# Domingo1337/Chiaroscuro-RayTracer

Measured on AMD Instinct MI355X. Metric: Mray/s (primary+secondary) on sponza_crytek 1080p; 1/2/4/8-GPU scaling, higher is better.
Workload: dtype f32; 1 GPU; sponza_standin (Sponza-Crytek stand-in, ~261k tris) 1920x1080; k=6, tile=32, parallelism=tile-split x1, rays=7648053528, rays_answered_untraced=1312885262, layers_per_pass=32, trace_build=59, texture_bytes=0

## Files before the change

### chiaroscuro-raytracer_amd/chiaroscuro_amd/__init__.py

```python
from __future__ import annotations

import ctypes as C
import os
from pathlib import Path

import numpy as np

PKG_ROOT = Path(__file__).resolve().parent.parent
LIB_DIR = Path(os.environ["CHIARO_LIB_DIR"]) if os.environ.get("CHIARO_LIB_DIR") else PKG_ROOT / "lib"

CR_OK = 0
CR_ERRORS = {-1: "CR_E_INVALID", -2: "CR_E_HIP", -3: "CR_E_NOSCENE", -4: "CR_E_DEPTH", -5: "CR_E_OOM",
             -6: "CR_E_COMM"}
COMM_ID_BYTES = 128

f3 = C.c_float * 3


class CrCamera(C.Structure):
    _fields_ = [("eye", f3), ("left_upper", f3), ("dx", f3), ("dy", f3)]

    def as_array(self) -> np.ndarray:
        return np.array(list(self.eye) + list(self.left_upper) + list(self.dx) + list(self.dy), dtype=np.float32)

# ... 68 lines not shown
    a = np.ascontiguousarray(x, np.float32)
    out = np.zeros(a.shape, np.uint16)
    libs()[1].chiaro_float_to_half(_ptr(a), out.ctypes.data_as(C.POINTER(C.c_uint16)), a.size)
    return out


class CrKdNode(C.Structure):
    _fields_ = [("split", C.c_float), ("axis", C.c_uint32), ("child_or_first", C.c_uint32), ("count", C.c_uint32)]


class CrTexture(C.Structure):
    _fields_ = [("width", C.c_int32), ("height", C.c_int32), ("components", C.c_int32),
                ("data", C.POINTER(C.c_uint8))]


class CrSceneDesc(C.Structure):
    _fields_ = [("n_nodes", C.c_uint32), ("nodes", C.POINTER(CrKdNode)), ("n_refs", C.c_uint32),
                ("refs", C.POINTER(C.c_uint32)), ("max_depth", C.c_uint32), ("box_min", f3), ("box_max", f3),
                ("n_tris", C.c_uint32), ("tri_pos", C.POINTER(C.c_float)), ("tri_normal", C.POINTER(C.c_float)),
                ("tri_kd", C.POINTER(C.c_float)), ("tri_ke", C.POINTER(C.c_float)),
                ("tri_uv", C.POINTER(C.c_float)), ("tri_tex", C.POINTER(C.c_int32)),
                ("tri_emissive", C.POINTER(C.c_uint8)), ("n_lights", C.c_uint32),
                ("light_id", C.POINTER(C.c_uint32)), ("light_surface", C.POINTER(C.c_float)),
                ("n_textures", C.c_uint32), ("textures", C.POINTER(CrTexture))]


class ChiaroSceneInfo(C.Structure):
    _fields_ = [("xres", C.c_uint32), ("yres", C.c_uint32), ("samples", C.c_uint32),
                ("preview_height", C.c_uint32), ("leaf_size", C.c_uint32), ("seed", C.c_uint32),
                ("k", C.c_int32), ("using_preview", C.c_int32), ("VP", f3), ("LA", f3), ("UP", f3),
                ("background", f3), ("yview", C.c_float), ("exposure", C.c_float), ("n_invalid", C.c_uint32),
                ("obj_path", C.c_char * 1024), ("render_path", C.c_char * 1024), ("gpus", C.c_uint32)]


TRACE_KINDS = ("camera", "closest", "shadow", "tail")
DIAG_NAMES = ("rounds", "lanes", "distinct", "records", "maxcount", "lanetests", "fit64", "fit128",
              "urounds", "tests", "geomiss", "rep1", "rep4", "rep8")
PERF_NAMES = ("queries", "steps", "leaves", "masks", "tests", "vbytes", "sbytes", "waves",
              "drounds", "diters", "dlanes", "dtests")


class CrTraceStats(C.Structure):
    _fields_ = [("launches", C.c_uint64 * 4), ("ms", C.c_double * 4), ("inner", C.c_uint64 * 4),
                ("leaf", C.c_uint64 * 4), ("tritest", C.c_uint64 * 4), ("chunked_shades", C.c_uint64)]


class CrTonemapParams(C.Structure):
    _fields_ = [(n, C.c_float) for n in ("m", "s", "kl", "f", "defog", "gamma")]


class CrNoiseParams(C.Structure):
    _fields_ = [("threshold", C.c_float), ("floor", C.c_float)]


class CrNoiseStats(C.Structure):
    _fields_ = [("pixels", C.c_uint64), ("above", C.c_uint64), ("max_err", C.c_float), ("layers", C.c_uint32)]

    def as_dict(self) -> dict:
        return {"pixels": int(self.pixels), "above": int(self.above), "max_err": float(self.max_err),
                "layers": int(self.layers)}


def tonemap_params(exposure, defog=0.0, knee_low=0.0, knee_high=5.0, gamma=2.2) -> CrTonemapParams:
    t = CrTonemapParams()
    libs()[0].cr_tonemap_setup(exposure, defog, knee_low, knee_high, gamma, C.byref(t))
    return t


_hip = None
_host = None

HIP_SYMBOLS = ("cr_create", "cr_destroy", "cr_last_error", "cr_upload_scene", "cr_render", "cr_render_device",
               "cr_render_tiles_device", "cr_blend_tiles_device", "cr_tiles_for_rank", "cr_tile_origin", "cr_intersect",
               "cr_intersect_shadow", "cr_intersect_device", "cr_intersect_shadow_device", "cr_get_counters", "cr_last_kernel_ms", "cr_get_trace_stats", "cr_set_option", "cr_synchronize", "cr_get_diag", "cr_get_perf", "cr_trace_build_available", "cr_last_trace_build",
               "cr_tonemap_setup", "cr_tonemap_device", "cr_tonemap",
               "cr_comm_unique_id", "cr_comm_init", "cr_comm_destroy", "cr_render_dist_device",
               "cr_device_count", "cr_group_create", "cr_group_destroy", "cr_group_last_error", "cr_group_size", "cr_group_ok",
               "cr_group_upload_scene", "cr_group_set_option", "cr_group_render", "cr_group_get_counters",
               "cr_group_rank_ms", "cr_group_ctx", "cr_group_tonemap", "cr_set_accumulator",
               "cr_group_set_accumulator", "cr_layers_per_pass", "cr_render_layers_device",
               "cr_render_tiles_layers_device", "cr_render_layers", "cr_scene_triangles", "cr_layers_per_group",
               "cr_blend_tiles_layers_device", "cr_render_dist_layers_device", "cr_group_render_layers",
               "cr_noise_struct_sizes", "cr_render_layers_noise_device", "cr_noise_device", "cr_render_layers_noise",
               "cr_noise", "cr_set_noise_accumulator", "cr_render_until")
HOST_SYMBOLS = ("chiaro_last_error", "chiaro_scene_create", "chiaro_scene_info_get", "chiaro_scene_destroy",
                "chiaro_model_create", "chiaro_model_load", "chiaro_model_num_meshes", "chiaro_model_num_triangles",
                "chiaro_model_num_textures", "chiaro_model_triangles", "chiaro_model_texture",
                "chiaro_model_destroy", "chiaro_kdtree_create", "chiaro_kdtree_num_nodes", "chiaro_kdtree_num_refs",
                "chiaro_kdtree_export", "chiaro_kdtree_describe", "chiaro_kdtree_destroy",
                "chiaro_raytracer_create", "chiaro_raytracer_raytrace", "chiaro_raytracer_raytrace_layers",
                "chiaro_raytracer_pixels",
                "chiaro_raytracer_data", "chiaro_raytracer_maxval", "chiaro_raytracer_layers",
                "chiaro_raytracer_counters", "chiaro_raytracer_normalize", "chiaro_raytracer_export",
                "chiaro_raytracer_ctx", "chiaro_raytracer_destroy", "chiaro_camera",
                "chiaro_raytracer_checkpoint", "chiaro_raytracer_resume", "chiaro_kdtree_fingerprint",
                "chiaro_checkpoint_write", "chiaro_checkpoint_read",
                "chiaro_exr_write", "chiaro_exr_write_half", "chiaro_exr_read_half", "chiaro_float_to_half",
                "chiaro_preview_create", "chiaro_preview_key", "chiaro_preview_mouse", "chiaro_preview_scroll",
                "chiaro_preview_texture", "chiaro_preview_state", "chiaro_preview_destroy",
                "chiaro_preview_camera_replay", "chiaro_raytracer_raytrace_until", "chiaro_raytracer_noise",
                "chiaro_raytracer_noise_map", "chiaro_noise_struct_sizes")

P = C.c_void_p
FP = C.POINTER(C.c_float)
UP = C.POINTER(C.c_uint32)


def _sig(lib, name, res, args):
    fn = getattr(lib, name)
    fn.restype = res
    fn.argtypes = args


def libs():
    global _hip, _host
    if _hip is not None:
        return _hip, _host
    hip_path, host_path = LIB_DIR / "libchiaro_hip.so", LIB_DIR / "libchiaroscuro.so"
    if not hip_path.exists() or not host_path.exists():
        raise RuntimeError("chiaroscuro_amd: native libraries not built (%s); run "
                           "`make -C chiaroscuro-raytracer_amd` or __graft_entry__.build()" % LIB_DIR)
    try:
        import torch
    except ImportError:
        pass
    hip = C.CDLL(str(hip_path), mode=C.RTLD_GLOBAL)
    host = C.CDLL(str(host_path))
    _sig(hip, "cr_create", P, [C.c_int])
    _sig(hip, "cr_destroy", None, [P])
    _sig(hip, "cr_last_error", C.c_char_p, [P])
    _sig(hip, "cr_upload_scene", C.c_int, [P, C.POINTER(CrSceneDesc)])
    _sig(hip, "cr_render", C.c_int, [P, C.POINTER(CrCamera), C.POINTER(CrRenderParams), FP])
    _sig(hip, "cr_render_device", C.c_int, [P, C.POINTER(CrCamera), C.POINTER(CrRenderParams), P, P])
    _sig(hip, "cr_render_tiles_device", C.c_int, [P, C.POINTER(CrCamera), C.POINTER(CrRenderParams), P, P])
    _sig(hip, "cr_layers_per_pass", C.c_uint32, [P, C.POINTER(CrRenderParams), C.c_uint32])
    _sig(hip, "cr_render_layers", C.c_int, [P, C.POINTER(CrCamera), C.POINTER(CrRenderParams), C.c_uint32, P])
    _sig(hip, "cr_scene_triangles", C.c_uint32, [P])
    _sig(hip, "cr_layers_per_group", C.c_uint32, [P, C.POINTER(CrRenderParams), C.c_uint32])
    _sig(hip, "cr_render_layers_device", C.c_int, [P, C.POINTER(CrCamera), C.POINTER(CrRenderParams), C.c_uint32, P, P])
    _sig(hip, "cr_render_tiles_layers_device", C.c_int,
         [P, C.POINTER(CrCamera), C.POINTER(CrRenderParams), C.c_uint32, P, P])
    _sig(hip, "cr_blend_tiles_device", C.c_int, [P, C.POINTER(CrRenderParams), P, P, P])
    _sig(hip, "cr_blend_tiles_layers_device", C.c_int, [P, C.POINTER(CrRenderParams), C.c_uint32, P, P, P])
    _sig(hip, "cr_tiles_for_rank", C.c_uint32, [C.POINTER(CrRenderParams), C.c_uint32])
    _sig(hip, "cr_tile_origin", C.c_int, [C.POINTER(CrRenderParams), C.c_uint32, C.c_uint32,
                                          C.POINTER(C.c_uint32), C.POINTER(C.c_uint32)])
    _sig(hip, "cr_intersect", C.c_int, [P, C.c_uint32, FP, FP, UP, UP, FP, FP])
    _sig(hip, "cr_intersect_shadow", C.c_int, [P, C.c_uint32, FP, FP, FP, UP, UP])
    _sig(hip, "cr_intersect_device", C.c_int, [P, C.c_uint32, P, P, P, P, P, P, P])
    _sig(hip, "cr_intersect_shadow_device", C.c_int, [P, C.c_uint32, P, P, P, P, P, P])
    _sig(hip, "cr_get_counters", C.c_int, [P, C.POINTER(CrCounters)])
    _sig(hip, "cr_last_kernel_ms", C.c_float, [P])
    _sig(hip, "cr_get_trace_stats", C.c_int, [P, C.POINTER(CrTraceStats)])
    _sig(hip, "cr_set_option", C.c_int, [P, C.c_char_p, C.c_int64])
    _sig(hip, "cr_get_diag", C.c_int, [P, C.POINTER(C.c_uint64), C.c_int])
    _sig(hip, "cr_get_perf", C.c_int, [P, C.POINTER(C.c_uint64), C.c_int])
    _sig(hip, "cr_trace_build_available", C.c_int, [C.c_int])
    _sig(hip, "cr_last_trace_build", C.c_int, [P])
    _sig(hip, "cr_synchronize", C.c_int, [P])
    _sig(hip, "cr_tonemap_setup", None, [C.c_float] * 5 + [C.POINTER(CrTonemapParams)])
    _sig(hip, "cr_tonemap_device", C.c_int, [P, C.POINTER(CrTonemapParams), C.c_uint32, C.c_uint32, P, P, P])
    _sig(hip, "cr_tonemap", C.c_int, [P, C.POINTER(CrTonemapParams), C.c_uint32, C.c_uint32,
                                      C.POINTER(C.c_uint8)])

    _sig(hip, "cr_comm_unique_id", C.c_int, [C.POINTER(C.c_uint8), C.c_size_t])
    _sig(hip, "cr_comm_init", C.c_int, [P, C.c_int, C.c_int, C.POINTER(C.c_uint8)])
    _sig(hip, "cr_comm_destroy", C.c_int, [P])
    _sig(hip, "cr_render_dist_device", C.c_int, [P, C.POINTER(CrCamera), C.POINTER(CrRenderParams), P, P])
    _sig(hip, "cr_render_dist_layers_device", C.c_int, [P, C.POINTER(CrCamera), C.POINTER(CrRenderParams),
                                                         C.c_uint32, P, P])
    _sig(hip, "cr_device_count", C.c_int, [])
    _sig(hip, "cr_group_create", P, [C.c_int, C.POINTER(C.c_int)])
    _sig(hip, "cr_group_destroy", None, [P])
    _sig(hip, "cr_group_last_error", C.c_char_p, [P])
    _sig(hip, "cr_group_size", C.c_int, [P])
    _sig(hip, "cr_group_ok", C.c_int, [P])
    _sig(hip, "cr_group_upload_scene", C.c_int, [P, C.POINTER(CrSceneDesc)])
    _sig(hip, "cr_group_set_option", C.c_int, [P, C.c_char_p, C.c_int64])
    _sig(hip, "cr_group_render", C.c_int, [P, C.POINTER(CrCamera), C.POINTER(CrRenderParams), FP])
    _sig(hip, "cr_group_render_layers", C.c_int, [P, C.POINTER(CrCamera), C.POINTER(CrRenderParams), C.c_uint32,
                                                   FP])
    _sig(hip, "cr_group_get_counters", C.c_int, [P, C.POINTER(CrCounters)])
    _sig(hip, "cr_group_rank_ms", C.c_int, [P, FP])
    _sig(hip, "cr_group_ctx", P, [P, C.c_int])
    _sig(hip, "cr_set_accumulator", C.c_int, [P, C.c_uint32, C.c_uint32, C.POINTER(C.c_float)])
    _sig(hip, "cr_group_set_accumulator", C.c_int, [P, C.c_uint32, C.c_uint32, C.POINTER(C.c_float)])
    _sig(hip, "cr_group_tonemap", C.c_int, [P, C.POINTER(CrTonemapParams), C.c_uint32, C.c_uint32,
                                            C.POINTER(C.c_uint8)])
    NP, NS = C.POINTER(CrNoiseParams), C.POINTER(CrNoiseStats)
    _sig(hip, "cr_noise_struct_sizes", None, [UP, UP])
    _sig(hip, "cr_render_layers_noise_device", C.c_int,
         [P, C.POINTER(CrCamera), C.POINTER(CrRenderParams), C.c_uint32, P, P, P])
    _sig(hip, "cr_noise_device", C.c_int, [P, C.c_uint32, C.c_uint32, C.c_uint32, C.c_uint32, NP, P, P, P, P, P])
    _sig(hip, "cr_render_layers_noise", C.c_int,
         [P, C.POINTER(CrCamera), C.POINTER(CrRenderParams), C.c_uint32, FP, FP])
    _sig(hip, "cr_noise", C.c_int, [P, C.c_uint32, C.c_uint32, C.c_uint32, C.c_uint32, NP, FP, NS])
    _sig(hip, "cr_set_noise_accumulator", C.c_int, [P, C.c_uint32, C.c_uint32, FP])
    _sig(hip, "cr_render_until", C.c_int, [P, C.POINTER(CrCamera), C.POINTER(CrRenderParams), C.c_uint32, C.c_uint32,
                                           C.c_uint32, NP, C.c_uint64, FP, NS])

    _sig(host, "chiaro_last_error", C.c_char_p, [])
    _sig(host, "chiaro_scene_create", P, [C.c_int, C.POINTER(C.c_char_p)])
    _sig(host, "chiaro_scene_info_get", C.c_int, [P, C.POINTER(ChiaroSceneInfo)])
    _sig(host, "chiaro_scene_destroy", None, [P])
    _sig(host, "chiaro_model_create", P, [P])
    _sig(host, "chiaro_model_load", P, [C.c_char_p])
    for n in ("chiaro_model_num_meshes", "chiaro_model_num_triangles", "chiaro_model_num_textures"):
        _sig(host, n, C.c_uint32, [P])
    _sig(host, "chiaro_model_triangles", C.c_int, [P, FP, FP, FP, FP, FP, C.POINTER(C.c_int32)])
    _sig(host, "chiaro_model_texture", C.c_int,
         [P, C.c_uint32, C.POINTER(C.c_int32), C.POINTER(C.c_int32), C.POINTER(C.c_int32),
          C.POINTER(C.POINTER(C.c_uint8))])
    _sig(host, "chiaro_model_destroy", None, [P])
    _sig(host, "chiaro_kdtree_create", P, [P, P, C.c_int])
    _sig(host, "chiaro_kdtree_num_nodes", C.c_uint32, [P])
    _sig(host, "chiaro_kdtree_num_refs", C.c_uint32, [P])
    _sig(host, "chiaro_kdtree_export", C.c_int, [P, UP, UP, FP, UP, UP, UP, UP, FP])
    _sig(host, "chiaro_kdtree_describe", C.c_int, [P, P, C.POINTER(CrSceneDesc)])
    _sig(host, "chiaro_kdtree_destroy", None, [P])
    _sig(host, "chiaro_raytracer_create", P, [P, P, C.c_int])
    _sig(host, "chiaro_raytracer_raytrace", C.c_int, [P, FP, FP, FP, C.c_float])
    _sig(host, "chiaro_raytracer_raytrace_layers", C.c_int, [P, C.c_uint32, FP, FP, FP, C.c_float])
    _sig(host, "chiaro_raytracer_raytrace_until", C.c_int, [P, C.c_float, C.c_uint32, FP, FP, FP, C.c_float, C.c_float,
                                                            C.c_uint32, C.c_uint64, UP])
# ... 193 lines not shown
        out = accum if accum is not None else np.zeros((p.yres, p.xres, 3), np.float32)
        assert out.dtype == np.float32 and out.flags.c_contiguous and out.size == p.yres * p.xres * 3
        self._chk(libs()[0].cr_render(self._c, C.byref(cam), C.byref(p), _ptr(out)), "cr_render")
        return out

    def render_layers(self, cam: CrCamera, p: CrRenderParams, nlayers: int,
                      accum: np.ndarray | None = None) -> np.ndarray:
        out = accum if accum is not None else np.zeros((p.yres, p.xres, 3), np.float32)
        assert out.dtype == np.float32 and out.flags.c_contiguous and out.size == p.yres * p.xres * 3
        self._chk(libs()[0].cr_render_layers(self._c, C.byref(cam), C.byref(p), nlayers, _ptr(out)),
                  "cr_render_layers")
        return out

    def render_layers_noise(self, cam: CrCamera, p: CrRenderParams, nlayers: int, accum: np.ndarray | None = None,
                            m2: np.ndarray | None = None):
        out = accum if accum is not None else np.zeros((p.yres, p.xres, 3), np.float32)
        mom = m2 if m2 is not None else np.zeros((p.yres, p.xres, 3), np.float32)
        for a in (out, mom):
            assert a.dtype == np.float32 and a.flags.c_contiguous and a.size == p.yres * p.xres * 3
        self._chk(libs()[0].cr_render_layers_noise(self._c, C.byref(cam), C.byref(p), int(nlayers), _ptr(out),
                                                   _ptr(mom)), "cr_render_layers_noise")
        return out, mom

    def render_layers_noise_device(self, cam, p, nlayers: int, d_frame_ptr: int, d_m2_ptr: int, stream: int = 0):
        self._chk(libs()[0].cr_render_layers_noise_device(self._c, C.byref(cam), C.byref(p), int(nlayers),
                                                          C.c_void_p(d_frame_ptr), C.c_void_p(d_m2_ptr),
                                                          C.c_void_p(stream)), "cr_render_layers_noise_device")

    def noise_device(self, xres: int, yres: int, layers: int, spp: int, threshold: float, floor: float,
                     d_frame_ptr: int, d_m2_ptr: int, d_err_ptr: int, d_stats_ptr: int, stream: int = 0):
        np_ = CrNoiseParams(float(threshold), float(floor))
        self._chk(libs()[0].cr_noise_device(self._c, int(xres), int(yres), int(layers), int(spp), C.byref(np_),
                                            C.c_void_p(d_frame_ptr), C.c_void_p(d_m2_ptr),
                                            C.c_void_p(d_err_ptr or None), C.c_void_p(d_stats_ptr),
                                            C.c_void_p(stream)), "cr_noise_device")

    def noise(self, xres: int, yres: int, layers: int, spp: int, threshold: float, floor: float,
              want_err: bool = True):
        np_ = CrNoiseParams(float(threshold), float(floor))
        st = CrNoiseStats()
        err = np.zeros((yres, xres), np.float32) if want_err else None
        self._chk(libs()[0].cr_noise(self._c, int(xres), int(yres), int(layers), int(spp), C.byref(np_),
                                     _ptr(err) if want_err else None, C.byref(st)), "cr_noise")
        return st.as_dict(), err

    def set_noise_accumulator(self, m2: np.ndarray):
        m2 = np.ascontiguousarray(m2, np.float32)
        self._chk(libs()[0].cr_set_noise_accumulator(self._c, m2.shape[1], m2.shape[0], _ptr(m2)),
                  "cr_set_noise_accumulator")

    def render_until(self, cam: CrCamera, p: CrRenderParams, min_layers: int, max_layers: int, check_every: int,
                     threshold: float, floor: float, max_above: int = 0, accum: np.ndarray | None = None):
        out = accum if accum is not None else np.zeros((p.yres, p.xres, 3), np.float32)
        assert out.dtype == np.float32 and out.flags.c_contiguous and out.size == p.yres * p.xres * 3
        np_ = CrNoiseParams(float(threshold), float(floor))
        st = CrNoiseStats()
        self._chk(libs()[0].cr_render_until(self._c, C.byref(cam), C.byref(p), int(min_layers), int(max_layers),
                                            int(check_every), C.byref(np_), int(max_above), _ptr(out), C.byref(st)),
                  "cr_render_until")
        return out, st.as_dict()

    def render_device(self, cam, p, d_frame_ptr: int, stream: int = 0):
        self._chk(libs()[0].cr_render_device(self._c, C.byref(cam), C.byref(p), C.c_void_p(d_frame_ptr),
                                             C.c_void_p(stream)), "cr_render_device")

    def render_tiles_device(self, cam, p, d_tiles_ptr: int, stream: int = 0):
        self._chk(libs()[0].cr_render_tiles_device(self._c, C.byref(cam), C.byref(p), C.c_void_p(d_tiles_ptr),
                                                   C.c_void_p(stream)), "cr_render_tiles_device")

    def layers_per_group(self, p, want: int) -> int:
        return int(libs()[0].cr_layers_per_group(self._c, C.byref(p), want))

    def scene_triangles(self) -> int:
        return int(libs()[0].cr_scene_triangles(self._c))

    def layers_per_pass(self, p, want: int) -> int:
        return int(libs()[0].cr_layers_per_pass(self._c, C.byref(p), want))

    def render_layers_device(self, cam, p, nlayers: int, d_frame_ptr: int, stream: int = 0):
        self._chk(libs()[0].cr_render_layers_device(self._c, C.byref(cam), C.byref(p), nlayers,
                                                    C.c_void_p(d_frame_ptr), C.c_void_p(stream)),
                  "cr_render_layers_device")

    def render_tiles_layers_device(self, cam, p, nlayers: int, d_tiles_ptr: int, stream: int = 0):
        self._chk(libs()[0].cr_render_tiles_layers_device(self._c, C.byref(cam), C.byref(p), nlayers,
                                                          C.c_void_p(d_tiles_ptr), C.c_void_p(stream)),
                  "cr_render_tiles_layers_device")

    def blend_tiles_layers_device(self, p, nlayers: int, d_gathered_ptr: int, d_frame_ptr: int, stream: int = 0):
        self._chk(libs()[0].cr_blend_tiles_layers_device(self._c, C.byref(p), int(nlayers), C.c_void_p(d_gathered_ptr),
                                                         C.c_void_p(d_frame_ptr), C.c_void_p(stream)),
                  "cr_blend_tiles_layers_device")

    def blend_tiles_device(self, p, d_gathered_ptr: int, d_frame_ptr: int, stream: int = 0):
        self._chk(libs()[0].cr_blend_tiles_device(self._c, C.byref(p), C.c_void_p(d_gathered_ptr),
                                                  C.c_void_p(d_frame_ptr), C.c_void_p(stream)),
                  "cr_blend_tiles_device")

    def tonemap_device(self, t: CrTonemapParams, xres: int, yres: int, d_rgb_ptr: int, d_bytes_ptr: int,
                       stream: int = 0):
        self._chk(libs()[0].cr_tonemap_device(self._c, C.byref(t), xres, yres, C.c_void_p(d_rgb_ptr),
                                              C.c_void_p(d_bytes_ptr), C.c_void_p(stream)), "cr_tonemap_device")

    @staticmethod
    def tiles_for_rank(p: CrRenderParams, rank: int) -> int:
        return int(libs()[0].cr_tiles_for_rank(C.byref(p), int(rank)))

    @staticmethod
    def tile_origin(p: CrRenderParams, rank: int, local: int):
        x0, y0 = C.c_uint32(0), C.c_uint32(0)
        if libs()[0].cr_tile_origin(C.byref(p), int(rank), int(local), C.byref(x0), C.byref(y0)):
            raise ValueError("cr_tile_origin: no such tile")
        return x0.value, y0.value

    def intersect_device(self, n: int, d_orig_ptr: int, d_dir_ptr: int, d_hit_ptr: int, d_tri_ptr: int = 0,
                         d_bary_ptr: int = 0, d_dist_ptr: int = 0, stream: int = 0):
        self._chk(libs()[0].cr_intersect_device(self._c, int(n), C.c_void_p(d_orig_ptr), C.c_void_p(d_dir_ptr),
                                                C.c_void_p(d_hit_ptr), C.c_void_p(d_tri_ptr or None),
                                                C.c_void_p(d_bary_ptr or None), C.c_void_p(d_dist_ptr or None),
                                                C.c_void_p(stream)), "cr_intersect_device")

    def intersect_shadow_device(self, n: int, d_orig_ptr: int, d_dir_ptr: int, d_dist_ptr: int, d_light_ptr: int,
                                d_occluded_ptr: int, stream: int = 0):
        self._chk(libs()[0].cr_intersect_shadow_device(self._c, int(n), C.c_void_p(d_orig_ptr), C.c_void_p(d_dir_ptr),
                                                       C.c_void_p(d_dist_ptr), C.c_void_p(d_light_ptr),
                                                       C.c_void_p(d_occluded_ptr), C.c_void_p(stream)),
                  "cr_intersect_shadow_device")

    def _query_tensor(self, t, dtype, shape, what):
        import torch
        if not (isinstance(t, torch.Tensor) and t.is_cuda and t.device.index == self.device and t.dtype == dtype and
                t.is_contiguous() and tuple(t.shape) == shape):
            raise ValueError("%s: a contiguous %s tensor of shape %s on cuda:%d is required" % (
                what, dtype, shape, self.device))
        return t

    def intersect_tensors(self, orig, dirs) -> dict:
        import torch
        n = int(orig.shape[0])
        self._query_tensor(orig, torch.float32, (n, 3), "orig")
        self._query_tensor(dirs, torch.float32, (n, 3), "dirs")
        hit = torch.zeros(n, dtype=torch.int32, device=orig.device)
        tri = torch.zeros(n, dtype=torch.int32, device=orig.device)
        bary = torch.zeros((n, 2), dtype=torch.float32, device=orig.device)
        dist = torch.zeros(n, dtype=torch.float32, device=orig.device)
        self.intersect_device(n, orig.data_ptr(), dirs.data_ptr(), hit.data_ptr(), tri.data_ptr(),
                              bary.data_ptr(), dist.data_ptr(), torch.cuda.current_stream(orig.device).cuda_stream)
        return {"hit": hit, "tri": tri, "bary": bary, "dist": dist}

    def intersect_shadow_tensors(self, orig, dirs, dist, light):
        import torch
        n = int(orig.shape[0])
        self._query_tensor(orig, torch.float32, (n, 3), "orig")
        self._query_tensor(dirs, torch.float32, (n, 3), "dirs")
        self._query_tensor(dist, torch.float32, (n,), "dist")
        self._query_tensor(light, torch.int32, (n,), "light")
        occ = torch.zeros(n, dtype=torch.int32, device=orig.device)
        self.intersect_shadow_device(n, orig.data_ptr(), dirs.data_ptr(), dist.data_ptr(), light.data_ptr(),
                                     occ.data_ptr(), torch.cuda.current_stream(orig.device).cuda_stream)
        return occ

    def intersect(self, orig: np.ndarray, dirs: np.ndarray) -> dict:
        orig = np.ascontiguousarray(orig, np.float32).reshape(-1, 3)
        dirs = np.ascontiguousarray(dirs, np.float32).reshape(-1, 3)
        n = len(orig)
        hit, tri = np.zeros(n, np.uint32), np.zeros(n, np.uint32)
# ... 294 lines not shown
```

### chiaroscuro-raytracer_amd/chiaroscuro_amd/tiles.py

```python
from __future__ import annotations

from dataclasses import dataclass


@dataclass(frozen=True)
class TileLayout:
    xres: int
    yres: int
    nranks: int = 1
    tile: int = 32

    @property
    def tiles_x(self) -> int:
        return (self.xres + self.tile - 1) // self.tile

    @property
    def tiles_y(self) -> int:
        return (self.yres + self.tile - 1) // self.tile

    @property
    def ntiles(self) -> int:
        return self.tiles_x * self.tiles_y

    def tiles_for_rank(self, rank: int) -> int:
# ... 9 lines not shown
        row, c = divmod(s, self.tiles_x)
        if self.nranks > 1:
            c = (c + row) % self.tiles_x
        return c * self.tile, row * self.tile


class DistributedFrame:

    def __init__(self, dev, xres: int, yres: int, rank: int, nranks: int, tile: int = 32, dist=None,
                 device: str = "cuda", gather: str = "torch"):
        import torch
        if nranks > 1 and (dist is None or dist.get_world_size() != nranks or dist.get_rank() != rank):
            raise ValueError("DistributedFrame: nranks %d / rank %d disagree with the process group" % (nranks, rank))
        if gather not in ("torch", "cabi"):
            raise ValueError("DistributedFrame: gather must be 'torch' or 'cabi'")
        self.dev, self.dist, self.rank, self.gather, self.device = dev, dist, rank, gather, device
        self.layout = TileLayout(xres, yres, nranks, tile)
        L = self.layout
        f32 = dict(dtype=torch.float32, device=device)
        self.frame = torch.zeros((yres, xres, 3), **f32) if rank == 0 or nranks == 1 else None
        split = nranks > 1 and gather == "torch"
        self.tiles = torch.zeros((L.max_tiles, tile, tile, 3), **f32) if split else None
        self.gathered = torch.zeros((nranks, L.max_tiles, tile, tile, 3), **f32) if split and rank == 0 else None
        self.tiles_multi = None
        self.gathered_multi = None
        self._stats_begin()
        if nranks > 1 and gather == "cabi":
            uid = [dev.comm_unique_id() if rank == 0 else None]
            dist.broadcast_object_list(uid, src=0)
            dev.comm_init(nranks, rank, uid[0])

    def save(self, path, header):
        if self.frame is None:
            return
        from . import checkpoint_write
        checkpoint_write(path, header, self.frame.cpu().numpy())

    def resume(self, path, expect) -> int:
        import torch
        layers = torch.zeros(1, dtype=torch.int64)
        err = ""
        if self.rank == 0:
            from . import checkpoint_read
            h, px = checkpoint_read(path)
            keys = ("xres", "yres", "samples", "k", "seed", "scene")
            if any(getattr(h, k) != getattr(expect, k) for k in keys) or list(h.background) != list(expect.background):
                err = "resume: the checkpoint is of another frame / sampling / scene"
            elif (list(h.eye) != list(expect.eye) or list(h.center) != list(expect.center)
                  or h.yview != expect.yview):
                err = "resume: the checkpoint is of another camera (eye / center / yview)"
            else:
                self.frame.copy_(torch.from_numpy(px).to(self.frame.device))
                layers[0] = h.layers
        if self.layout.nranks > 1:
            flag = torch.tensor([0 if not err else 1], dtype=torch.int64)
            if self.dist.get_backend() == "nccl":
                layers, flag = layers.cuda(), flag.cuda()
            self.dist.broadcast(layers, src=0)
            self.dist.broadcast(flag, src=0)
            if int(flag.item()):
                err = err or "resume: rank 0 refused the checkpoint"
        if err:
            raise ValueError(err)
        return int(layers.item())

    def plan_layers(self, params, want: int):
        L = self.layout
        want = max(1, int(want))
        if not hasattr(self.dev, "layers_per_pass"):
            return 1, 1
        if L.nranks > 1:
            n = self.dev.layers_per_group(params, want) if hasattr(self.dev, "layers_per_group") \
                else self.dev.layers_per_pass(params, want)
            import torch
            t = torch.tensor([n], dtype=torch.int64, device=self.device)
            self.dist.all_reduce(t, op=self.dist.ReduceOp.MIN)
            return int(t.item()), 1
        max_pieces = min(64, L.ntiles)
        if hasattr(self.dev, "scene_triangles") and self.dev.scene_triangles() < 1024:
            max_pieces = 1
        for nl in range(want, 0, -1):
            for m in range(1, max_pieces + 1):
                q = _with_layer(params, params.layer)
                q.rank, q.nranks = 0, m
                if self.dev.layers_per_pass(q, nl) == nl:
                    return nl, m
        return 1, 1

    def reserve(self, nlayers: int):
        import torch
        L = self.layout
        if L.nranks == 1 or self.gather != "torch" or nlayers < 2:
            return
        if self.tiles_multi is None or self.tiles_multi.shape[0] < nlayers:
            self.tiles_multi = torch.zeros((nlayers,) + tuple(self.tiles.shape), dtype=self.tiles.dtype,
                                           device=self.tiles.device)
        if self.rank == 0:
            self._gathered_view(nlayers)

    def _gathered_view(self, nlayers: int):
        import torch
        shape = (self.layout.nranks, nlayers) + tuple(self.tiles.shape)
        n = 1
        for x in shape:
            n *= x
        if self.gathered_multi is None or self.gathered_multi.numel() < n:
            self.gathered_multi = torch.zeros(n, dtype=self.tiles.dtype, device=self.tiles.device)
        return self.gathered_multi[:n].view(shape)

    def render_layers(self, cam, params, nlayers: int, stream: int = 0, pieces: int = 1):
        import torch
        L = self.layout
        self._stats_begin()
        if nlayers == 1 and pieces == 1:
            self._render_one(cam, params, stream)
            return
        if (params.rank, params.nranks, params.tile or 32, params.xres, params.yres) != \
                (self.rank, L.nranks, L.tile, L.xres, L.yres):
            raise ValueError("render_layers: params do not match this frame's partition")
        if L.nranks == 1:
            for k in range(pieces):
                q = _with_layer(params, params.layer)
                q.rank, q.nranks = k, pieces
                self.dev.render_layers_device(cam, q, nlayers, self.frame.data_ptr(), stream)
                self._stats_add()
            return
        if pieces != 1:
            raise ValueError("render_layers: frame pieces on a single rank only")
        if self.gather == "cabi":
            self.dev.render_dist_layers_device(cam, params, nlayers, self.frame.data_ptr() if self.rank == 0 else 0,
                                               stream)
            self._stats_add()
            return
        if self.tiles_multi is None or self.tiles_multi.shape[0] < nlayers:
            self.tiles_multi = torch.zeros((nlayers,) + tuple(self.tiles.shape), dtype=self.tiles.dtype,
                                           device=self.tiles.device)
        mine = self.tiles_multi[:nlayers]
        self.dev.render_tiles_layers_device(cam, params, nlayers, mine.data_ptr(), stream)
        self._stats_add()
        if not hasattr(self.dev, "blend_tiles_layers_device"):
            for j in range(nlayers):
                self.dist.gather(mine[j], [self.gathered[r] for r in range(L.nranks)] if self.rank == 0 else None,
                                 dst=0)
                if self.rank == 0:
                    self.dev.blend_tiles_device(_with_layer(params, params.layer + j), self.gathered.data_ptr(),
                                                self.frame.data_ptr(), stream)
            return
        g = self._gathered_view(nlayers) if self.rank == 0 else None
        self.dist.gather(mine, [g[r] for r in range(L.nranks)] if self.rank == 0 else None, dst=0)
        if self.rank == 0:
            self.dev.blend_tiles_layers_device(params, nlayers, g.data_ptr(), self.frame.data_ptr(), stream)

    def _stats_begin(self):
        self._stats = {"counters": {}, "kernel_ms": 0.0, "trace": None, "passes": 0}

    def _stats_add(self):
        st = self._stats
        st["passes"] += 1
        if not hasattr(self.dev, "counters"):
            return
        for key, v in self.dev.counters().items():
            st["counters"][key] = st["counters"].get(key, 0) + v
        st["kernel_ms"] += self.dev.last_kernel_ms()
        if hasattr(self.dev, "trace_stats"):
            ts = self.dev.trace_stats()
            if st["trace"] is None:
                st["trace"] = {k: dict(v) for k, v in ts.items()}
            else:
                for kind, v in ts.items():
                    for key, x in v.items():
                        st["trace"][kind][key] += x

    def last_stats(self):
        return self._stats

    def _render_one(self, cam, params, stream):
        self.render_layer(cam, params, stream, _keep_stats=True)

    def render_layer(self, cam, params, stream: int = 0, _keep_stats: bool = False):
        if not _keep_stats:
            self._stats_begin()
        L = self.layout
        if (params.rank, params.nranks, params.tile or 32, params.xres, params.yres) != \
                (self.rank, L.nranks, L.tile, L.xres, L.yres):
            raise ValueError("render_layer: params do not match this frame's partition")
        if L.nranks == 1:
            self.dev.render_device(cam, params, self.frame.data_ptr(), stream)
            self._stats_add()
            return
        if self.gather == "cabi":
            self.dev.render_dist_device(cam, params, self.frame.data_ptr() if self.rank == 0 else 0, stream)
            self._stats_add()
            return
        self.dev.render_tiles_device(cam, params, self.tiles.data_ptr(), stream)
        self._stats_add()
        self.dist.gather(self.tiles, [self.gathered[r] for r in range(L.nranks)] if self.rank == 0 else None, dst=0)
        if self.rank == 0:
            self.dev.blend_tiles_device(params, self.gathered.data_ptr(), self.frame.data_ptr(), stream)


def _with_layer(params, layer: int):
    q = type(params).from_buffer_copy(params)
    q.layer = layer
    return q
```

### chiaroscuro-raytracer_amd/csrc/cabi.cpp

```cpp
#include "ctx.hpp"
#include "leafcull.hpp"
#include "wfplan.hpp"

#include <algorithm>
#include <cmath>
#include <cstdio>
#include <cstring>
#include <string>
#include <thread>
#include <vector>

namespace crx {

int fail(cr_ctx *c, int code, const std::string &msg) {
    if (c) c->err = msg;
    return code;
}
int hip_fail(cr_ctx *c, hipError_t e, const char *what) {
    return fail(c, CR_E_HIP, std::string(what) + ": " + hipGetErrorString(e));
}


void free_scene(cr_ctx *c) {
    for (void *p : c->scene_bufs) hipFree(p);
    c->scene_bufs.clear();
    c->has_scene = false;
    c->S = cr::DevScene{};
    c->d_levels = nullptr;
    c->levels.clear();
}

template <class T> int upload(cr_ctx *c, const std::vector<T> &h, const T **out) {
    void *d = nullptr;
    size_t bytes = h.size() * sizeof(T);
    if (bytes == 0) bytes = 16;
    hipError_t e = hipMalloc(&d, bytes);
    if (e != hipSuccess) return fail(c, CR_E_OOM, std::string("hipMalloc: ") + hipGetErrorString(e));
    c->scene_bufs.push_back(d);
    if (!h.empty()) {
        e = hipMemcpy(d, h.data(), h.size() * sizeof(T), hipMemcpyHostToDevice);
        if (e != hipSuccess) return hip_fail(c, e, "hipMemcpy(scene)");
    }
    *out = (const T *)d;
    return CR_OK;
}

int check_params(cr_ctx *c, const cr_render_params *p) {
    if (!p) return fail(c, CR_E_INVALID, "null params");
    if (!c->has_scene) return fail(c, CR_E_NOSCENE, "no scene uploaded");
    if (p->xres == 0 || p->yres == 0 || p->spp == 0) return fail(c, CR_E_INVALID, "xres/yres/spp must be > 0");
    if (p->k < 1 || p->k > 64) return fail(c, CR_E_INVALID, "k must be in [1, 64]");
    if (p->layer < 1) return fail(c, CR_E_INVALID, "layer must be >= 1");
    if (p->nranks < 1 || p->rank >= p->nranks) return fail(c, CR_E_INVALID, "bad rank/nranks");
    uint64_t px = (uint64_t)p->xres * p->yres;
    if (px > (1ull << 31)) return fail(c, CR_E_INVALID, "image too large");
    return CR_OK;
}

uint32_t tile_of(const cr_render_params *p) { return p->tile ? p->tile : 32u; }

int grow(cr_ctx *c, void **buf, size_t &cap, size_t need) {
    if (need <= cap && *buf) return CR_OK;
    if (*buf) hipFree(*buf);
    *buf = nullptr;
    cap = 0;
    if (hipMalloc(buf, need ? need : 16) != hipSuccess) return fail(c, CR_E_OOM, "work buffer");
    cap = need;
    return CR_OK;
}

using cr::LEAF_CULL_MIN_TRIS;
using cr::SORT_MIN_TRIS;

int default_trace_build(const cr_ctx *c) { return cr::wf_default_build(c->n_tris); }

void fill_trace_tuning(const cr_ctx *c, cr::RenderArgs &A) {
    A.lc_min = c->lc_min;
    A.desc_quorum = c->desc_quorum >= 0 ? (uint32_t)c->desc_quorum
                    : ((c->n_tris >= SORT_MIN_TRIS && c->n_tris < LEAF_CULL_MIN_TRIS) ? 0u : 8u);
    A.refill = c->refill ? c->refill : 48u;
    A.refill_shadow = c->refill_shadow ? c->refill_shadow
                                       : (c->refill ? c->refill : (c->n_tris >= SORT_MIN_TRIS ? 60u : 56u));
    A.refill_camera = c->refill_camera ? c->refill_camera : (c->refill ? c->refill : 64u);
}

void fill_args(cr_ctx *c, cr::RenderArgs &A, const cr_camera *cam, const cr_render_params *p, float *out, int mode) {
    A.S = c->S;
    std::memcpy(A.cam, cam->eye, 3 * sizeof(float));
    std::memcpy(A.cam + 3, cam->left_upper, 3 * sizeof(float));
    std::memcpy(A.cam + 6, cam->dx, 3 * sizeof(float));
    std::memcpy(A.cam + 9, cam->dy, 3 * sizeof(float));
    A.xres = p->xres;
    A.yres = p->yres;
    A.spp = p->spp;
    A.K = p->k;
    A.bg[0] = p->background[0];
    A.bg[1] = p->background[1];
    A.bg[2] = p->background[2];
    A.seed = p->seed;
    A.layer = p->layer;
    A.nl = 1;
    A.layer_stride = 0;
    A.piece_k = 0;
    A.piece_m = 1;
    A.rank = p->rank;
    A.nranks = p->nranks;
    A.tile = tile_of(p);
    A.tiles_x = (p->xres + A.tile - 1) / A.tile;
    A.n_items = cr_tiles_for_rank(p, p->rank) * A.tile * A.tile;
    A.stack_depth = c->stack_depth;
    A.mode = mode;
    A.out = out;
    A.counters = c->d_counters;
    A.full_counters = c->full_counters;
    A.perf_counters = c->perf_counters;
    A.diag_kinds = c->diag_kinds;
    A.lc_debug = c->lc_debug;
    fill_trace_tuning(c, A);
    A.variant = c->variant >= 0 ? c->variant : default_trace_build(c);
    A.eye_on_split = 0;
    for (int a = 0; a < 3; a++)
        if (std::binary_search(c->splits[a].begin(), c->splits[a].end(), cam->eye[a])) A.eye_on_split = 1;
}

uint64_t wf_path_cap(cr_ctx *c, int k) {
    if (!c->wf_mem_budget) {
        size_t freeb = 0, totalb = 0;
        if (hipMemGetInfo(&freeb, &totalb) != hipSuccess) return ~0ull;
        c->wf_mem_budget = freeb + c->wf_bytes + c->wf2_bytes;
    }
    return cr::wf_path_cap_of(c->wf_mem_budget, k, cr::wf_chunked(*c, c->n_tris));
}

cr_counters counters_of(const unsigned long long *h) {
    return cr_counters{h[0], h[1],  h[2],  h[3],  h[4],  h[5],  h[6],  h[7], h[8],
                       h[9], h[10], h[11], h[12], h[13], h[14], h[15], h[16],
                       h[17], h[18], h[19], h[20], h[21], h[cr::CTR_NEE]};
}

int run_render(cr_ctx *c, const cr_camera *cam, const cr_render_params *p, float *out, int mode, hipStream_t st,
               uint32_t nl, uint32_t piece_k, uint32_t piece_m, uint64_t stride, float *m2) {
    if (!cam || !out) return fail(c, CR_E_INVALID, "null camera/output");
    if (m2 && mode != cr::MODE_BLEND) return fail(c, CR_E_INVALID, "moments are tracked for blended frames only");
    int rc = check_params(c, p);
    if (rc) return rc;
    if (nl < 1 || (nl > 1 && (c->kernel != 2 || c->wf_lanes != 1)))
        return fail(c, CR_E_INVALID, "layers per pass: >= 1, and > 1 only with the wavefront kernel in one lane");
    HIPCHK(hipSetDevice(c->device));
    cr::RenderArgs A{};
    fill_args(c, A, cam, p, out, mode);
    A.nl = nl;
    A.layer_stride = (uint64_t)cr_tiles_for_rank(p, 0) * A.tile * A.tile * 3;
    if (piece_m > 1) {
        if (mode != cr::MODE_TILES || piece_k >= piece_m || !stride) return fail(c, CR_E_INVALID, "bad piece");
        A.piece_k = piece_k;
        A.piece_m = piece_m;
        A.layer_stride = stride;
    }
    if (c->kernel == 2 && !c->full_counters && !cr::wf_variant_available(A.variant))
        return fail(c, CR_E_INVALID, "trace build " + std::to_string(A.variant) +
                                         " does not exist (DESIGN.md §3 lists the measured builds that were removed)");
    if (c->perf_counters && (c->kernel != 2 || c->full_counters || !cr::wf_perf_available(A.variant)))
        return fail(c, CR_E_INVALID, "perf_counters: the wavefront kernel's trace builds " + cr::wf_perf_builds_text() +
                                         " only, without the counting build");
    c->last_build = c->kernel == 2 ? (c->full_counters ? -1 : A.variant) : -2;
    HIPCHK(hipMemsetAsync(c->d_counters, 0, cr::CTR_SLOTS * sizeof(unsigned long long), st));
    uint32_t blk, blocks;
    cr::wf_trace_geometry(c->full_counters ? -1 : A.variant, c->num_cus, blk, blocks);
    A.gstride = blk * blocks;
    const uint32_t shade_blocks = c->wf_app_chunk ? cr::wf_shade_blocks(c->num_cus, c->wf_shade_waves) : 0u;
    const cr::WfPlanIn in{*c, A.n_items, p->spp, nl, p->k, A.tile, c->n_tris, A.S.n_nodes, c->stack_depth, A.gstride,
                          shade_blocks, wf_path_cap(c, p->k)};
    const cr::WfPlan pl = cr::wf_plan(in);
    if (pl.code) return fail(c, pl.code, pl.msg);
    const int lanes = c->wf_lanes;
    if (int r = grow(c, &c->d_gstack, c->gstack_bytes, pl.gstack_bytes)) return r;
    if (int r = grow(c, &c->d_samples, c->samples_bytes, pl.samples_bytes)) return r;
    if (pl.chunked)
        if (int r = grow(c, &c->d_run, c->run_bytes, pl.run_bytes)) return r;
    if (pl.chunked && m2)
        if (int r = grow(c, &c->d_run2, c->run2_bytes, pl.run_bytes)) return r;
    if (int r = grow(c, &c->d_wf, c->wf_bytes, pl.need_alloc)) return r;
    if (lanes == 2)
        if (int r = grow(c, &c->d_wf2, c->wf2_bytes, pl.need_alloc)) return r;
    A.gstack = (uint2 *)c->d_gstack;
    A.samples = (float *)c->d_samples;
    A.run = (float *)c->d_run;
    cr::WfArgs W{};
    cr::WfArgs W2{};
    cr::wf_bind(in, pl, c->d_wf, A.gstack, 0, W);
    if (lanes == 2) cr::wf_bind(in, pl, c->d_wf2, A.gstack, 1, W2);
    const bool cull = !c->full_counters && cr::wf_variant_culls(A.variant);
    if (cull) {
        if (int r = grow(c, &c->d_cull, c->cull_bytes, 16 * ((size_t)c->n_refs + 4))) return r;
        if (int r = grow(c, &c->d_cull_node, c->cull_node_bytes, 16 * (size_t)c->S.n_nodes)) return r;
    }
    A.cull = cull ? (const float4 *)c->d_cull : nullptr;
    A.cull_node = cull ? (const float4 *)c->d_cull_node : nullptr;
    c->tev.n = 0;
    c->tev.chunked = 0;
    HIPCHK(hipEventRecord(c->ev0, st));
    if (cull)
        if (int e = cr::launch_cam_cull(A, c->n_refs, (float4 *)c->d_cull, (float4 *)c->d_cull_node, c->d_levels,
                                        (const uint32_t(*)[2])c->levels.data(), (int)c->levels.size(), st))
            return hip_fail(c, (hipError_t)e, "cull-box kernel launch");
    for (uint32_t s0 = 0; s0 < pl.spp_pass; s0 += (uint32_t)pl.chunk) {
        A.s0 = s0;
        A.s_count = (uint32_t)std::min<uint64_t>(pl.chunk, pl.spp_pass - s0);
        A.n_work = A.n_items * A.s_count;
        int e = 0;
        if (lanes == 2) {
            cr::WfLane L[2] = {{W, st, c->wfs.side, c->wfs.fork, c->wfs.join, c->lane_ev[0], c->hcnt},
                               {W2, c->stream2, c->side2, c->fork2, c->join2, c->lane_ev[1], c->hcnt + 2}};
            e = cr::run_wavefront_lanes(A, L, 2, c->num_cus, st, &c->tev);
        } else {
            const uint32_t P = W.P;
            for (uint32_t w0 = 0; w0 < A.n_work && !e; w0 += P) {
                W.w0 = w0;
                W.P = std::min(P, A.n_work - w0);
                HIPCHK(hipMemsetAsync(W.cnt, 0, cr::WF_CNT * sizeof(uint32_t), st));
                e = cr::launch_wavefront_chunk(A, W, c->num_cus, st, c->wfs, &c->tev);
            }
            W.P = P;
        }
        if (!e) e = cr::launch_sum_samples(A, s0 == 0, s0 + A.s_count == pl.spp_pass, st, c->sum_lds, c->sum_staged != 0,
                                            m2, (float *)c->d_run2);
        if (e) return hip_fail(c, (hipError_t)e, "render kernel launch");
    }
    HIPCHK(hipEventRecord(c->ev1, st));
    unsigned long long h[cr::CTR_SLOTS];
    HIPCHK(hipMemcpyAsync(h, c->d_counters, sizeof(h), hipMemcpyDeviceToHost, st));
    HIPCHK(hipStreamSynchronize(st));
    HIPCHK(hipEventElapsedTime(&c->last_ms, c->ev0, c->ev1));
    c->last = counters_of(h);
    for (int i = 0; i < cr::DIAG_N; i++) c->last_diag[i] = h[cr::CTR_DIAG + i];
    for (int i = 0; i < cr::TK_N * cr::PERF_N; i++) c->last_perf[i] = h[cr::CTR_PERF + i];
    c->last_trace = cr_trace_stats{};
    if (c->kernel == 2) {
        for (int i = 0; i < c->tev.n; i++) {
            float ms = 0.f;
            HIPCHK(hipEventElapsedTime(&ms, c->tev.ev[2 * i], c->tev.ev[2 * i + 1]));
            const int k = c->tev.kind[i];
            c->last_trace.launches[k]++;
            c->last_trace.ms[k] += ms;
        }
        c->last_trace.chunked_shades = (uint64_t)c->tev.chunked;
        for (int k = 0; k < cr::TK_TAIL; k++) {
            c->last_trace.inner[k] = h[cr::CTR_TRACE + 3 * k];
            c->last_trace.leaf[k] = h[cr::CTR_TRACE + 3 * k + 1];
            c->last_trace.tritest[k] = h[cr::CTR_TRACE + 3 * k + 2];
        }
    }
    return CR_OK;
}

}

using namespace crx;

extern "C" {

cr_ctx *cr_create(int device) {
    cr_ctx *c = new cr_ctx();
    int n = 0;
    if (hipGetDeviceCount(&n) != hipSuccess || n <= 0) {
        c->err = "no HIP device";
        return c;
    }
    if (device < 0 || device >= n) {
        c->err = "bad device index";
        return c;
    }
    c->device = device;
    if (hipSetDevice(device) != hipSuccess) {
        c->err = "hipSetDevice failed";
        c->device = -1;
        return c;
    }
    hipDeviceProp_t prop;
    if (hipGetDeviceProperties(&prop, device) == hipSuccess) c->num_cus = prop.multiProcessorCount;
    if (hipStreamCreateWithFlags(&c->stream, hipStreamNonBlocking) != hipSuccess ||
        hipStreamCreateWithFlags(&c->wfs.side, hipStreamNonBlocking) != hipSuccess ||
        hipEventCreateWithFlags(&c->wfs.fork, hipEventDisableTiming) != hipSuccess ||
        hipEventCreateWithFlags(&c->wfs.join, hipEventDisableTiming) != hipSuccess ||
        hipStreamCreateWithFlags(&c->stream2, hipStreamNonBlocking) != hipSuccess ||
        hipStreamCreateWithFlags(&c->side2, hipStreamNonBlocking) != hipSuccess ||
        hipEventCreateWithFlags(&c->fork2, hipEventDisableTiming) != hipSuccess ||
        hipEventCreateWithFlags(&c->join2, hipEventDisableTiming) != hipSuccess ||
        hipEventCreateWithFlags(&c->lane_ev[0], hipEventDisableTiming) != hipSuccess ||
        hipEventCreateWithFlags(&c->lane_ev[1], hipEventDisableTiming) != hipSuccess ||
        hipHostMalloc((void **)&c->hcnt, 4 * sizeof(uint32_t), hipHostMallocDefault) != hipSuccess ||
        hipEventCreate(&c->ev0) != hipSuccess || hipEventCreate(&c->ev1) != hipSuccess ||
        hipEventCreateWithFlags(&c->q_ev, hipEventDisableTiming) != hipSuccess ||
        hipMalloc(&c->d_counters, cr::CTR_SLOTS * sizeof(unsigned long long)) != hipSuccess) {
        c->err = "device init failed";
        c->device = -1;
    }
    return c;
}

void cr_destroy(cr_ctx *c) {
    if (!c) return;
    if (c->device >= 0) {
        hipSetDevice(c->device);
        release_dist(c);
        free_scene(c);
        if (c->d_accum) hipFree(c->d_accum);
        if (c->d_gstack) hipFree(c->d_gstack);
        if (c->d_samples) hipFree(c->d_samples);
        if (c->d_run) hipFree(c->d_run);
        if (c->d_accum2) hipFree(c->d_accum2);
        if (c->d_run2) hipFree(c->d_run2);
        if (c->d_err) hipFree(c->d_err);
        if (c->d_nstats) hipFree(c->d_nstats);
        if (c->d_wf) hipFree(c->d_wf);
        if (c->d_cull) hipFree(c->d_cull);
        if (c->d_cull_node) hipFree(c->d_cull_node);
        if (c->d_counters) hipFree(c->d_counters);
        if (c->ev0) hipEventDestroy(c->ev0);
        for (int i = 0; i < 2 * c->tev.cap; i++) hipEventDestroy(c->tev.ev[i]);
        delete[] c->tev.ev;
        delete[] c->tev.kind;
        if (c->ev1) hipEventDestroy(c->ev1);
        if (c->stream) hipStreamDestroy(c->stream);
        if (c->wfs.side) hipStreamDestroy(c->wfs.side);
        if (c->wfs.fork) hipEventDestroy(c->wfs.fork);
        if (c->wfs.join) hipEventDestroy(c->wfs.join);
        if (c->stream2) hipStreamDestroy(c->stream2);
        if (c->side2) hipStreamDestroy(c->side2);
        if (c->fork2) hipEventDestroy(c->fork2);
        if (c->join2) hipEventDestroy(c->join2);
        for (hipEvent_t e : c->lane_ev)
            if (e) hipEventDestroy(e);
        if (c->hcnt) hipHostFree(c->hcnt);
        if (c->d_wf2) hipFree(c->d_wf2);
        if (c->q_pending) hipEventSynchronize(c->q_ev);
        if (c->d_query) hipFree(c->d_query);
        if (c->q_ev) hipEventDestroy(c->q_ev);
    }
    delete c;
}

const char *cr_last_error(cr_ctx *c) { return c ? c->err.c_str() : "null context"; }

int cr_upload_scene(cr_ctx *c, const cr_scene_desc *d) {
    if (!c) return CR_E_INVALID;
    if (c->device < 0) return fail(c, CR_E_HIP, c->err.empty() ? "no device" : c->err);
    if (!d || !d->nodes || d->n_nodes == 0) return fail(c, CR_E_INVALID, "empty kd tree");
    if (d->n_tris && (!d->tri_pos || !d->tri_normal || !d->tri_kd || !d->tri_ke || !d->tri_uv))
        return fail(c, CR_E_INVALID, "missing triangle arrays");
    if (d->max_depth > 256) return fail(c, CR_E_DEPTH, "kd tree deeper than 256");
    HIPCHK(hipSetDevice(c->device));
    free_scene(c);
    c->wf_mem_budget = 0;
    const uint32_t nt = d->n_tris;
    const uint32_t NN = d->n_nodes;
    for (uint32_t i = 0; i < NN; i++) {
        const cr_kdnode &n = d->nodes[i];
        if (n.axis == 3) {
            if (n.count >= (1u << 30) || (uint64_t)n.child_or_first + n.count > d->n_refs)
                return fail(c, CR_E_INVALID, "bad leaf range");
        } else if (n.axis > 2 || (uint64_t)n.child_or_first + 1 >= NN || n.child_or_first >= (1u << 30)) {
            return fail(c, CR_E_INVALID, "bad inner node");
        }
    }
    std::vector<uint32_t> newid(NN, 0xffffffffu), order;
    order.reserve(NN);
    order.push_back(0);
    newid[0] = 0;
    for (size_t h = 0; h < order.size() && order.size() + 2 <= c->node_bfs; h++) {
        const cr_kdnode &n = d->nodes[order[h]];
        if (n.axis == 3) continue;
        for (uint32_t k = 0; k < 2; k++) {
            const uint32_t ch = n.child_or_first + k;
            if (newid[ch] != 0xffffffffu) return fail(c, CR_E_INVALID, "kd node with two parents");
            newid[ch] = (uint32_t)order.size();
            order.push_back(ch);
        }
    }
    for (uint32_t i = 0; i < NN; i++)
        if (newid[i] == 0xffffffffu) {
            newid[i] = (uint32_t)order.size();
            order.push_back(i);
        }
    std::vector<uint2> nodes(NN);
    for (uint32_t i = 0; i < NN; i++) {
        const cr_kdnode &n = d->nodes[i];
        if (n.axis == 3) {
            nodes[newid[i]] = make_uint2(n.child_or_first, 3u | (n.count << 2));
        } else {
            const uint32_t ch = newid[n.child_or_first];
            if (newid[n.child_or_first + 1] != ch + 1) return fail(c, CR_E_INVALID, "kd siblings not adjacent");
            uint32_t sb;
            std::memcpy(&sb, &n.split, 4);
            nodes[newid[i]] = make_uint2(sb, n.axis | (ch << 2));
        }
    }
    if ((uint64_t)32 * d->n_nodes > 0xFFFFFFFFull) return fail(c, CR_E_INVALID, "more than 134 M kd nodes");
    std::vector<uint4> fat((size_t)2 * d->n_nodes, make_uint4(0u, 0u, 0u, 0u));
    for (uint32_t i = 0; i < d->n_nodes; i++) {
// ... 175 lines not shown
    return CR_OK;
}

int cr_tile_origin(const cr_render_params *p, uint32_t rank, uint32_t local, uint32_t *x0, uint32_t *y0) {
    if (!p || !x0 || !y0 || local >= cr_tiles_for_rank(p, rank)) return CR_E_INVALID;
    const uint32_t T = tile_of(p), tx = (p->xres + T - 1) / T, s = rank + local * p->nranks;
    *x0 = cr::tile_slot_column(s, tx, p->nranks) * T;
    *y0 = s / tx * T;
    return CR_OK;
}

uint32_t cr_tiles_for_rank(const cr_render_params *p, uint32_t rank) {
    if (!p || p->nranks == 0 || rank >= p->nranks || p->xres == 0 || p->yres == 0) return 0;
    const uint32_t T = tile_of(p);
    const uint32_t nt = ((p->xres + T - 1) / T) * ((p->yres + T - 1) / T);
    return nt > rank ? (nt - rank + p->nranks - 1) / p->nranks : 0;
}

static int size_accumulator(cr_ctx *c, size_t elems, bool zero) {
    if (elems == c->accum_elems) return CR_OK;
    if (c->d_accum) hipFree(c->d_accum);
    c->d_accum = nullptr;
    c->accum_elems = 0;
    if (hipMalloc(&c->d_accum, elems * sizeof(float)) != hipSuccess) return fail(c, CR_E_OOM, "accumulator");
    c->accum_elems = elems;
    if (zero) HIPCHK(hipMemset(c->d_accum, 0, elems * sizeof(float)));
    return CR_OK;
}
static int size_noise_accumulator(cr_ctx *c, size_t elems, bool zero) {
    if (elems == c->accum2_elems) return CR_OK;
    if (c->d_accum2) hipFree(c->d_accum2);
    c->d_accum2 = nullptr;
    c->accum2_elems = 0;
    if (hipMalloc(&c->d_accum2, elems * sizeof(float)) != hipSuccess) return fail(c, CR_E_OOM, "moment accumulator");
    c->accum2_elems = elems;
    if (zero) HIPCHK(hipMemset(c->d_accum2, 0, elems * sizeof(float)));
    return CR_OK;
}

int cr_render(cr_ctx *c, const cr_camera *cam, const cr_render_params *p, float *accum_rgb_out) {
    if (!c) return CR_E_INVALID;
    if (c->device < 0) return fail(c, CR_E_HIP, c->err.empty() ? "no device" : c->err);
    if (!accum_rgb_out || !p) return fail(c, CR_E_INVALID, "null output/params");
    cr_render_params q = *p;
    if (q.nranks == 0) q.nranks = 1;
    int rc = check_params(c, &q);
    if (rc) return rc;
    HIPCHK(hipSetDevice(c->device));
    const size_t elems = (size_t)q.xres * q.yres * 3;
    if (int r = size_accumulator(c, elems, true)) return r;
    rc = run_render(c, cam, &q, c->d_accum, cr::MODE_BLEND, c->stream);
    if (rc) return rc;
    HIPCHK(hipMemcpy(accum_rgb_out, c->d_accum, elems * sizeof(float), hipMemcpyDeviceToHost));
    return CR_OK;
}


static const uint32_t LAYER_GROUP = 32, MAX_PIECES = 64;
static const uint32_t PIECES_MIN_TRIS = 1024;
uint32_t cr_scene_triangles(cr_ctx *c) { return c && c->has_scene ? c->n_tris : 0u; }
}
uint32_t crx::group_layers(cr_ctx *c, const cr_render_params *p, uint32_t want, uint32_t *m_out) {
    *m_out = 1;
    const uint32_t N = p->nranks ? p->nranks : 1;
    const uint32_t share = cr_tiles_for_rank(p, p->rank);
    const uint32_t maxm = c->n_tris < PIECES_MIN_TRIS ? 1u : std::min(MAX_PIECES, std::max(share, 1u));
    for (uint32_t nl = std::max(want, 1u); nl > 1; nl--)
        for (uint32_t m = 1; m <= maxm; m++) {
            cr_render_params t = *p;
            t.nranks = N * m;
            t.rank = N == 1 ? 0 : p->rank;
            if (cr_layers_per_pass(c, &t, nl) == nl) {
                *m_out = m;
                return nl;
            }
        }
    return 1;
}
static int render_layer_group(cr_ctx *c, const cr_camera *cam, const cr_render_params &g, uint32_t want, float *m2,
                              crx::PassTotals &sum, uint32_t *nl_out) {
    uint32_t m = 1;
    const uint32_t nl = crx::group_layers(c, &g, std::min(LAYER_GROUP, want), &m);
    for (uint32_t k = 0; k < m; k++) {
        cr_render_params t = g;
        t.rank = k;
        t.nranks = m;
        if (int rc = crx::run_render(c, cam, &t, c->d_accum, cr::MODE_BLEND, c->stream, nl, 0, 1, 0, m2)) return rc;
        sum.add(c);
    }
    *nl_out = nl;
    return CR_OK;
}
static int render_layer_groups(cr_ctx *c, const cr_camera *cam, const cr_render_params &q, uint32_t nlayers, float *m2,
                               crx::PassTotals &sum) {
    for (uint32_t done = 0, nl = 0; done < nlayers; done += nl) {
        cr_render_params g = q;
        g.layer = q.layer + done;
        if (int rc = render_layer_group(c, cam, g, nlayers - done, m2, sum, &nl)) return rc;
    }
    return CR_OK;
}
extern "C" {

uint32_t cr_layers_per_group(cr_ctx *c, const cr_render_params *p, uint32_t want) {
    if (!c || c->device < 0 || !c->has_scene || !p || want < 1 || check_params(c, p) != CR_OK) return 1;
    uint32_t m = 1;
    return group_layers(c, p, want, &m);
}

int cr_render_layers(cr_ctx *c, const cr_camera *cam, const cr_render_params *p, uint32_t nlayers,
                     float *accum_rgb_out) {
    if (!c) return CR_E_INVALID;
    if (c->device < 0) return fail(c, CR_E_HIP, c->err.empty() ? "no device" : c->err);
    if (!accum_rgb_out || !p || nlayers < 1) return fail(c, CR_E_INVALID, "null output/params or no layers");
    cr_render_params q = *p;
    if (q.nranks == 0) q.nranks = 1;
    if (q.nranks != 1) return fail(c, CR_E_INVALID, "cr_render_layers: the whole frame (nranks 1)");
    int rc = check_params(c, &q);
    if (rc) return rc;
    HIPCHK(hipSetDevice(c->device));
    const size_t elems = (size_t)q.xres * q.yres * 3;
    if (int r = size_accumulator(c, elems, true)) return r;
    PassTotals sum;
    if ((rc = render_layer_groups(c, cam, q, nlayers, nullptr, sum))) return rc;
    sum.store(c);
    HIPCHK(hipMemcpy(accum_rgb_out, c->d_accum, elems * sizeof(float), hipMemcpyDeviceToHost));
    return CR_OK;
}

int cr_set_accumulator(cr_ctx *c, uint32_t xres, uint32_t yres, const float *rgb) {
    if (!c) return CR_E_INVALID;
    if (c->device < 0) return fail(c, CR_E_HIP, c->err.empty() ? "no device" : c->err);
    if (!rgb || !xres || !yres) return fail(c, CR_E_INVALID, "null / empty accumulator");
    HIPCHK(hipSetDevice(c->device));
    const size_t elems = (size_t)xres * yres * 3;
    if (int r = size_accumulator(c, elems, false)) return r;
    HIPCHK(hipMemcpy(c->d_accum, rgb, elems * sizeof(float), hipMemcpyHostToDevice));
    return CR_OK;
}

}
static int check_noise_params(cr_ctx *c, const cr_noise_params *np) {
    if (!np) return fail(c, CR_E_INVALID, "null noise params");
    if (!(np->floor > 0.f) || std::isinf(np->floor)) return fail(c, CR_E_INVALID, "noise floor must be > 0 and finite");
    if (!(np->threshold >= 0.f)) return fail(c, CR_E_INVALID, "noise threshold must be >= 0");
    return CR_OK;
}
static int check_noise_shape(cr_ctx *c, uint32_t xres, uint32_t yres, uint32_t layers, uint32_t spp) {
    if (!xres || !yres || !layers || !spp) return fail(c, CR_E_INVALID, "xres/yres/layers/spp must be > 0");
    if ((uint64_t)xres * yres > (1ull << 31)) return fail(c, CR_E_INVALID, "image too large");
    if ((uint64_t)layers * spp > 0xFFFFFFFFull) return fail(c, CR_E_INVALID, "layers * spp must fit 32 bits");
    return CR_OK;
}
static int enqueue_noise(cr_ctx *c, uint32_t xres, uint32_t yres, uint32_t layers, uint32_t spp,
                         const cr_noise_params *np, const float *d_frame, const float *d_m2, float *d_err,
                         cr_noise_stats *d_stats, hipStream_t st) {
    HIPCHK(hipSetDevice(c->device));
    HIPCHK(hipMemsetAsync(d_stats, 0, sizeof(cr_noise_stats), st));
    cr::NoiseArgs N{};
    N.frame = d_frame;
    N.m2 = d_m2;
    N.err = d_err;
    N.stats = d_stats;
    N.npix = xres * yres;
    N.layers = layers;
    N.n = (float)(layers * spp);
    N.threshold = np->threshold;
    N.floor = np->floor;
    if (int e = cr::launch_noise_eval(N, st)) return hip_fail(c, (hipError_t)e, "noise kernel launch");
    return CR_OK;
// ... 73 lines not shown
    if (c->device < 0) return fail(c, CR_E_HIP, c->err.empty() ? "no device" : c->err);
    return noise_of_accumulators(c, xres, yres, layers, spp, np, err_out, stats_out);
}

int cr_set_noise_accumulator(cr_ctx *c, uint32_t xres, uint32_t yres, const float *m2) {
    if (!c) return CR_E_INVALID;
    if (!m2 || !xres || !yres) return fail(c, CR_E_INVALID, "null / empty moment accumulator");
    if (c->device < 0) return fail(c, CR_E_HIP, c->err.empty() ? "no device" : c->err);
    HIPCHK(hipSetDevice(c->device));
    const size_t elems = (size_t)xres * yres * 3;
    if (int r = size_noise_accumulator(c, elems, false)) return r;
    HIPCHK(hipMemcpy(c->d_accum2, m2, elems * sizeof(float), hipMemcpyHostToDevice));
    return CR_OK;
}

int cr_render_until(cr_ctx *c, const cr_camera *cam, const cr_render_params *p, uint32_t min_layers,
                    uint32_t max_layers, uint32_t check_every, const cr_noise_params *np, uint64_t max_above,
                    float *accum_rgb_out, cr_noise_stats *stats_out) {
    if (!c) return CR_E_INVALID;
    if (!cam || !p || !accum_rgb_out || !stats_out) return fail(c, CR_E_INVALID, "null camera/params/output/stats");
    if (int r = check_noise_params(c, np)) return r;
    if (check_every < 1 || p->layer < 1 || max_layers < p->layer)
        return fail(c, CR_E_INVALID, "cr_render_until: check_every >= 1 and 1 <= p->layer <= max_layers");
    if (c->device < 0) return fail(c, CR_E_HIP, c->err.empty() ? "no device" : c->err);
    cr_render_params q = *p;
    if (q.nranks == 0) q.nranks = 1;
    if (q.nranks != 1) return fail(c, CR_E_INVALID, "cr_render_until: the whole frame (nranks 1)");
    int rc = check_params(c, &q);
    if (rc) return rc;
    if ((rc = check_noise_shape(c, q.xres, q.yres, max_layers, q.spp))) return rc;
    HIPCHK(hipSetDevice(c->device));
    const size_t elems = (size_t)q.xres * q.yres * 3;
    if (int r = size_accumulator(c, elems, true)) return r;
    if (int r = size_noise_accumulator(c, elems, true)) return r;
    PassTotals sum;
    cr_noise_stats st{};
    for (uint32_t layer = q.layer - 1; layer < max_layers;) {
        uint32_t n = 0;
        cr_render_params g = q;
        g.layer = layer + 1;
        if ((rc = render_layer_group(c, cam, g, std::min(check_every, max_layers - layer), c->d_accum2, sum, &n)))
            return rc;
        layer += n;
        if ((rc = noise_of_accumulators(c, q.xres, q.yres, layer, q.spp, np, nullptr, &st))) return rc;
        if (layer >= min_layers && st.above <= max_above) break;
    }
    sum.store(c);
    HIPCHK(hipMemcpy(accum_rgb_out, c->d_accum, elems * sizeof(float), hipMemcpyDeviceToHost));
    *stats_out = st;
    return CR_OK;
}

int cr_render_device(cr_ctx *c, const cr_camera *cam, const cr_render_params *p, float *d_frame, void *stream) {
    if (!c) return CR_E_INVALID;
    if (c->device < 0) return fail(c, CR_E_HIP, c->err.empty() ? "no device" : c->err);
    return run_render(c, cam, p, d_frame, cr::MODE_BLEND, (hipStream_t)stream);
}

int cr_render_tiles_device(cr_ctx *c, const cr_camera *cam, const cr_render_params *p, float *d_tiles,
                           void *stream) {
    if (!c) return CR_E_INVALID;
    if (c->device < 0) return fail(c, CR_E_HIP, c->err.empty() ? "no device" : c->err);
    return run_render(c, cam, p, d_tiles, cr::MODE_TILES, (hipStream_t)stream);
}

uint32_t cr_layers_per_pass(cr_ctx *c, const cr_render_params *p, uint32_t want) {
    if (!c || c->device < 0 || !c->has_scene || !p || want < 1 || check_params(c, p) != CR_OK) return 1;
    if (c->kernel != 2 || c->wf_lanes != 1 || c->full_counters) return 1;
    if (hipSetDevice(c->device) != hipSuccess) return 1;
    const uint64_t items = (uint64_t)cr_tiles_for_rank(p, p->rank) * tile_of(p) * tile_of(p);
    const uint64_t paths_cap = std::min<uint64_t>(c->wf_paths, wf_path_cap(c, p->k));
    uint32_t nl = want;
    while (nl > 1 && !cr::wf_layers_fit(items, p->spp, nl, paths_cap, c->sample_buf)) nl--;
    return nl;
}

int cr_render_layers_device(cr_ctx *c, const cr_camera *cam, const cr_render_params *p, uint32_t nlayers,
                            float *d_frame, void *stream) {
    if (!c) return CR_E_INVALID;
    if (c->device < 0) return fail(c, CR_E_HIP, c->err.empty() ? "no device" : c->err);
    return run_render(c, cam, p, d_frame, cr::MODE_BLEND, (hipStream_t)stream, nlayers);
}

int cr_render_tiles_layers_device(cr_ctx *c, const cr_camera *cam, const cr_render_params *p, uint32_t nlayers,
                                  float *d_tiles, void *stream) {
    if (!c) return CR_E_INVALID;
    if (c->device < 0) return fail(c, CR_E_HIP, c->err.empty() ? "no device" : c->err);
    if (!p || p->nranks <= 1 || nlayers <= 1 || cr_layers_per_pass(c, p, nlayers) == nlayers)
        return run_render(c, cam, p, d_tiles, cr::MODE_TILES, (hipStream_t)stream, nlayers);
    uint32_t m = 1;
    if (group_layers(c, p, nlayers, &m) != nlayers)
        return fail(c, CR_E_INVALID, "layers per pass: the rank's share does not fit in pieces");
    const uint64_t stride = (uint64_t)cr_tiles_for_rank(p, 0) * tile_of(p) * tile_of(p) * 3;
    PassTotals sum;
    for (uint32_t k = 0; k < m; k++) {
        cr_render_params t = *p;
        t.rank = p->rank + k * p->nranks;
        t.nranks = p->nranks * m;
        if (cr_tiles_for_rank(&t, t.rank) == 0) continue;
        if (int rc = run_render(c, cam, &t, d_tiles, cr::MODE_TILES, (hipStream_t)stream, nlayers, k, m, stride))
            return rc;
        sum.add(c);
    }
    sum.store(c);
    return CR_OK;
}

int cr_blend_tiles_device(cr_ctx *c, const cr_render_params *p, const float *d_gathered, float *d_frame,
                          void *stream) {
    return cr_blend_tiles_layers_device(c, p, 1, d_gathered, d_frame, stream);
}

int cr_blend_tiles_layers_device(cr_ctx *c, const cr_render_params *p, uint32_t nlayers, const float *d_gathered,
                                 float *d_frame, void *stream) {
    if (!c) return CR_E_INVALID;
    if (c->device < 0) return fail(c, CR_E_HIP, c->err.empty() ? "no device" : c->err);
    if (!p || !d_gathered || !d_frame || p->nranks < 1 || p->layer < 1 || nlayers < 1)
        return fail(c, CR_E_INVALID, "bad blend args");
    HIPCHK(hipSetDevice(c->device));
    cr::BlendArgs B{};
    B.gathered = d_gathered;
    B.frame = d_frame;
    B.xres = p->xres;
    B.yres = p->yres;
    B.tile = tile_of(p);
    B.tiles_x = (p->xres + B.tile - 1) / B.tile;
    B.nranks = p->nranks;
    B.max_tiles = cr_tiles_for_rank(p, 0);
    B.layer = p->layer;
    B.nl = nlayers;
    int e = cr::launch_blend(B, (hipStream_t)stream);
    if (e) return hip_fail(c, (hipError_t)e, "blend kernel launch");
    return CR_OK;
}

static inline float tm_knee(double x, double f) { return logf(x * f + 1) / f; }
static float tm_find_knee_f(float x, float y) {
    float f0 = 0, f1 = 1;
    while (tm_knee(x, f1) > y) {
        f0 = f1;
        f1 = f1 * 2;
    }
    for (int i = 0; i < 30; ++i) {
        const float f2 = (f0 + f1) / 2;
        if (tm_knee(x, f2) < y) f1 = f2;
        else f0 = f2;
    }
    return (f0 + f1) / 2;
}

void cr_tonemap_setup(float exposure, float defog, float kneeLow, float kneeHigh, float gamma, cr_tonemap_params *t) {
    if (!t) return;
    t->m = powf(2.f, exposure + 2.47393f);
    t->s = 255.f * powf(2.f, -3.5f * gamma);
    t->kl = powf(2.f, kneeLow);
    t->f = tm_find_knee_f(powf(2.f, kneeHigh), powf(2.f, 3.5) - t->kl);
    t->defog = defog;
    t->gamma = gamma;
}

int cr_tonemap_device(cr_ctx *c, const cr_tonemap_params *t, uint32_t xres, uint32_t yres, const float *d_rgb,
                      uint8_t *d_bytes, void *stream) {
    if (!c) return CR_E_INVALID;
    if (c->device < 0) return fail(c, CR_E_HIP, c->err.empty() ? "no device" : c->err);
    if (!t || !d_rgb || !d_bytes) return fail(c, CR_E_INVALID, "bad tonemap args");
    if ((uint64_t)xres * yres > (1ull << 31)) return fail(c, CR_E_INVALID, "image too large");
    HIPCHK(hipSetDevice(c->device));
    const cr::TonemapArgs T{d_rgb, d_bytes, xres, yres, t->m, t->s, t->kl, t->f, t->defog, t->gamma};
    const int e = cr::launch_tonemap(T, (hipStream_t)stream);
    if (e) return hip_fail(c, (hipError_t)e, "tonemap kernel launch");
    return CR_OK;
}

int cr_tonemap(cr_ctx *c, const cr_tonemap_params *t, uint32_t xres, uint32_t yres, uint8_t *bytes_out) {
    if (!c) return CR_E_INVALID;
    if (c->device < 0) return fail(c, CR_E_HIP, c->err.empty() ? "no device" : c->err);
    if (!bytes_out) return fail(c, CR_E_INVALID, "null output");
    const size_t n = (size_t)3 * xres * yres;
    if (!c->d_accum || c->accum_elems != n) return fail(c, CR_E_INVALID, "no rendered frame of this size");
    HIPCHK(hipSetDevice(c->device));
    void *d_bytes = nullptr;
    if (hipMalloc(&d_bytes, n ? n : 1) != hipSuccess) return fail(c, CR_E_OOM, "tonemap buffer");
    int rc = cr_tonemap_device(c, t, xres, yres, c->d_accum, (uint8_t *)d_bytes, c->stream);
    if (rc == CR_OK) {
// ... 234 lines not shown
                               const uint32_t *d_light_tri, uint32_t *d_occluded, void *stream) {
    return run_query_device(c, n, true, d_orig, d_dir, d_dist, d_light_tri, d_occluded, nullptr, nullptr, nullptr,
                            stream);
}

int cr_get_counters(cr_ctx *c, cr_counters *out) {
    if (!c || !out) return CR_E_INVALID;
    *out = c->last;
    return CR_OK;
}

float cr_last_kernel_ms(cr_ctx *c) { return c ? c->last_ms : 0.f; }

int cr_get_trace_stats(cr_ctx *c, cr_trace_stats *out) {
    if (!c || !out) return CR_E_INVALID;
    *out = c->last_trace;
    return CR_OK;
}

int cr_trace_build_available(int build) { return cr::wf_variant_available(build) ? 1 : 0; }
int cr_last_trace_build(cr_ctx *c) { return c ? c->last_build : -2; }

int cr_get_diag(cr_ctx *c, uint64_t *out, int n) {
    if (!c || !out || n < 0) return CR_E_INVALID;
    for (int i = 0; i < n && i < cr::DIAG_N; i++) out[i] = c->last_diag[i];
    return CR_OK;
}

int cr_get_perf(cr_ctx *c, uint64_t *out, int n) {
    if (!c || !out || n < 0) return CR_E_INVALID;
    for (int i = 0; i < n && i < cr::TK_N * cr::PERF_N; i++) out[i] = c->last_perf[i];
    return CR_OK;
}

int cr_set_option(cr_ctx *c, const char *key, int64_t v) {
    if (!c || !key) return CR_E_INVALID;
    const int64_t nvar = cr::num_wf_variants();
    if (!std::strcmp(key, "kernel") && v == 2) c->kernel = (int)v;
    else if (!std::strcmp(key, "counters") && (v == 0 || v == 1)) c->full_counters = (int)v;
    else if (!std::strcmp(key, "perf_counters") && (v == 0 || v == 1)) c->perf_counters = (int)v;
    else if (!std::strcmp(key, "wf_tail_overlap") && (v == 0 || v == 1)) c->wf_tail_overlap = (int)v;
    else if (!std::strcmp(key, "wf_sort_g1") && v >= 0 && v <= 3) c->wf_sort_g1 = (uint32_t)v;
    else if (!std::strcmp(key, "wf_cam_lean") && (v == 0 || v == 1)) c->wf_cam_lean = (int)v;
    else if (!std::strcmp(key, "wf_cam_fuse") && (v == 0 || v == 1)) c->wf_cam_fuse = (int)v;
    else if (!std::strcmp(key, "wf_ctl_ray") && (v == 0 || v == 1)) c->wf_ctl_ray = (int)v;
    else if (!std::strcmp(key, "wf_vis_dw") && (v == 0 || v == 1)) c->wf_vis_dw = (int)v;
    else if (!std::strcmp(key, "wf_vis_mark") && (v == 0 || v == 1)) c->wf_vis_mark = (int)v;
    else if (!std::strcmp(key, "sum_lds") && v >= 0 && v <= 65536) c->sum_lds = (uint32_t)v;
    else if (!std::strcmp(key, "wf_nee_skip") && (v == 0 || v == 1)) c->wf_nee_skip = (int)v;
    else if (!std::strcmp(key, "sum_staged") && (v == 0 || v == 1)) c->sum_staged = (int)v;
    else if (!std::strcmp(key, "wf_tail_waves") && v >= 4 && v <= 6) c->wf_tail_waves = (int)v;
    else if (!std::strcmp(key, "wf_side_priority") && (v == 0 || v == 1)) {
        int lo = 0, hi = 0;
        if (hipSetDevice(c->device) != hipSuccess || hipDeviceSynchronize() != hipSuccess ||
            hipDeviceGetStreamPriorityRange(&lo, &hi) != hipSuccess)
            return CR_E_HIP;
        hipStream_t s = nullptr;
        if (hipStreamCreateWithPriority(&s, hipStreamNonBlocking, v ? hi : lo) != hipSuccess) return CR_E_HIP;
        hipStreamDestroy(c->wfs.side);
        c->wfs.side = s;
    }
    else if (!std::strcmp(key, "diag_kinds") && v >= 0 && v <= 7) c->diag_kinds = (uint32_t)v;
    else if (!std::strcmp(key, "lc_debug") && v >= 0 && v <= 2) c->lc_debug = (int)v;
    else if (!std::strcmp(key, "lc_min") && v >= 0 && v <= 33) c->lc_min = (uint32_t)v;
    else if (!std::strcmp(key, "desc_quorum") && v >= -1 && v <= 64) c->desc_quorum = (int)v;
    else if (!std::strcmp(key, "comm_timeout_ms") && v >= 1 && v <= 3600000) c->comm_timeout_ms = (uint32_t)v;
    else if (!std::strcmp(key, "variant") && v >= -1 && v < nvar) c->variant = (int)v;
    else if (!std::strcmp(key, "refill") && v >= 0 && v <= 64) c->refill = (uint32_t)v;
    else if (!std::strcmp(key, "refill_shadow") && v >= 0 && v <= 64) c->refill_shadow = (uint32_t)v;
    else if (!std::strcmp(key, "refill_camera") && v >= 0 && v <= 64) c->refill_camera = (uint32_t)v;
    else if (!std::strcmp(key, "wf_sort") && v >= -1 && v <= 1) c->wf_sort = (int)v;
    else if (!std::strcmp(key, "wf_world_keys") && v >= 0 && v <= 64) c->wf_world_keys = (int)v;
    else if (!std::strcmp(key, "wf_world_bits") && v >= 1 && v <= 10) c->wf_world_bits = (uint32_t)v;
    else if (!std::strcmp(key, "wf_sort_min") && v >= 0 && v <= (1ll << 31)) c->wf_sort_min = (uint32_t)v;
    else if (!std::strcmp(key, "wf_tail_min") && v >= 0 && v <= 0xffffffffll) c->wf_tail_min = (uint32_t)v;
    else if (!std::strcmp(key, "wf_sort_tile") && v >= 0 && v <= 5) c->wf_sort_tile = (uint32_t)v;
    else if (!std::strcmp(key, "wf_dir_res") && v >= 1 && v <= 256 && (v & (v - 1)) == 0)
        c->wf_dir_res = (uint32_t)v;
    else if (!std::strcmp(key, "wf_dir_res_shadow") && v >= 0 && v <= 256 && (v & (v - 1)) == 0)
        c->wf_dir_res_shadow = (uint32_t)v;
    else if (!std::strcmp(key, "wf_paths") && v >= 4096 && v <= (1ll << 30)) c->wf_paths = (uint32_t)v;
    else if (!std::strcmp(key, "wf_lanes") && (v == 1 || v == 2)) c->wf_lanes = (int)v;
    else if (!std::strcmp(key, "wf_xcd") && v >= 0 && v <= 7) c->wf_xcd = (uint32_t)v;
    else if (!std::strcmp(key, "wf_leaf_keys") && (v == 0 || v == 1)) c->wf_leaf_keys = (int)v;
    else if (!std::strcmp(key, "wf_resolve_paths") && v >= 0 && v <= 64) c->wf_resolve_paths = (uint32_t)v;
    else if (!std::strcmp(key, "wf_measure_skip") && v >= 0 && v <= 3) c->wf_measure_skip = (uint32_t)v;
    else if (!std::strcmp(key, "wf_shade_waves") && (v == 6 || v == 8)) c->wf_shade_waves = (int)v;
    else if (!std::strcmp(key, "wf_shade_block") && (v == 256 || v == 512 || v == 1024)) c->wf_shade_block = (int)v;
    else if (!std::strcmp(key, "wf_app_chunk") && (v == 0 || (v >= 256 && v <= 65536 && !(v & (v - 1))))) c->wf_app_chunk = (int)v;
    else if (!std::strcmp(key, "wf_leaf_shift") && v >= 0 && v <= 24) c->wf_leaf_shift = (uint32_t)v;
    else if (!std::strcmp(key, "node_bfs") && v >= 1 && v <= (1ll << 30)) c->node_bfs = (uint32_t)v;
    else if (!std::strcmp(key, "sample_buf_bytes") && v >= 1 && v <= (1ll << 40)) c->sample_buf = (uint64_t)v;
    else if (!std::strcmp(key, "query_route") && v >= 0 && v <= 2) c->query_route = (int)v;
    else if (!std::strcmp(key, "query_sort") && v >= -1 && v <= 1) c->query_sort = (int)v;
    else if (!std::strcmp(key, "query_chunk") && v >= 256 && v <= (1ll << 24)) c->query_chunk = (uint32_t)v;
    else if (!std::strcmp(key, "query_trace_min") && v >= 0 && v <= 0xffffffffll) c->query_trace_min = (uint32_t)v;
    else return fail(c, CR_E_INVALID, std::string("unknown option or value: ") + key);
    return CR_OK;
}

int cr_synchronize(cr_ctx *c) {
    if (!c) return CR_E_INVALID;
    if (c->device < 0) return fail(c, CR_E_HIP, "no device");
    HIPCHK(hipSetDevice(c->device));
    HIPCHK(hipDeviceSynchronize());
    return CR_OK;
}

}
```

### chiaroscuro-raytracer_amd/csrc/ctx.hpp

```cpp
#pragma once
#include "chiaro_hip.h"
#include "kernels.hpp"
#include "wfopts.hpp"

#include <hip/hip_runtime.h>
#include <rccl/rccl.h>

#include <cstring>
#include <string>
#include <vector>

struct cr_ctx : cr::WfOptions {
    int device = -1;
    int num_cus = 0;
    std::string err;
    hipStream_t stream = nullptr;
    hipEvent_t ev0 = nullptr, ev1 = nullptr;
    cr::WfStreams wfs{nullptr, nullptr, nullptr};
    hipStream_t stream2 = nullptr, side2 = nullptr;
    hipEvent_t fork2 = nullptr, join2 = nullptr, lane_ev[2] = {nullptr, nullptr};
    uint32_t *hcnt = nullptr;
    void *d_wf2 = nullptr;
    size_t wf2_bytes = 0;
    uint64_t wf_mem_budget = 0;
    float last_ms = 0.f;
    int last_build = -2;
    bool has_scene = false;
    cr::DevScene S{};
    uint32_t stack_depth = 1;
    uint32_t n_refs = 0;
    uint32_t n_tris = 0;
    std::vector<float> splits[3];
    const uint32_t *d_levels = nullptr;
    std::vector<std::pair<uint32_t, uint32_t>> levels;
    std::vector<void *> scene_bufs;
    unsigned long long *d_counters = nullptr;
    float *d_accum = nullptr;
    size_t accum_elems = 0;
    void *d_gstack = nullptr, *d_samples = nullptr, *d_run = nullptr, *d_wf = nullptr;
    size_t gstack_bytes = 0, samples_bytes = 0, run_bytes = 0, wf_bytes = 0;
    float *d_accum2 = nullptr;
    size_t accum2_elems = 0;
    void *d_run2 = nullptr, *d_err = nullptr, *d_nstats = nullptr;
    size_t run2_bytes = 0, err_bytes = 0, nstats_bytes = 0;
    void *d_cull = nullptr;
    size_t cull_bytes = 0;
    void *d_cull_node = nullptr;
    size_t cull_node_bytes = 0;
    cr_counters last{};
    cr::TraceEvents tev;
    cr_trace_stats last_trace{};
    int kernel = 2;
    int full_counters = 1;
    int lc_debug = 0;
    uint32_t lc_min = 0;
    int desc_quorum = -1;
    uint32_t diag_kinds = 0;
    unsigned long long last_diag[cr::DIAG_N] = {};
    int perf_counters = 0;
    unsigned long long last_perf[cr::TK_N * cr::PERF_N] = {};
    int variant = -1;
    uint32_t refill = 0;
    uint32_t refill_shadow = 0;
    uint32_t refill_camera = 0;
    uint32_t sum_lds = 0;
    int sum_staged = 1;
    uint32_t node_bfs = cr::NODE_BFS;
    ncclComm_t comm = nullptr;
    int comm_rank = 0, comm_nranks = 1;
    uint32_t comm_timeout_ms = 120000;
    float *d_tiles = nullptr, *d_gathered = nullptr;
    size_t tiles_bytes = 0, gathered_bytes = 0;
    int *d_flag = nullptr;
    size_t flag_bytes = 0;
    void *d_query = nullptr;
    size_t query_bytes = 0;
    uint32_t q_cap = 0, q_depth = 0;
    bool q_trace = false;
    hipEvent_t q_ev = nullptr;
    bool q_pending = false;
    hipStream_t q_stream = nullptr;
    int query_route = 0;
    int query_sort = -1;
    uint32_t query_chunk = 1u << 24;
    uint32_t query_trace_min = 1u << 16;
};


#define HIPCHK(call)                                                                                                 \
    do {                                                                                                             \
        hipError_t e_ = (call);                                                                                      \
        if (e_ != hipSuccess) return crx::hip_fail(c, e_, #call);                                                    \
    } while (0)

namespace crx {
int fail(cr_ctx *c, int code, const std::string &msg);
int hip_fail(cr_ctx *c, hipError_t e, const char *what);
int check_params(cr_ctx *c, const cr_render_params *p);
uint32_t tile_of(const cr_render_params *p);
int grow(cr_ctx *c, void **buf, size_t &cap, size_t need);
int run_render(cr_ctx *c, const cr_camera *cam, const cr_render_params *p, float *out, int mode, hipStream_t st,
               uint32_t nl = 1, uint32_t piece_k = 0, uint32_t piece_m = 1, uint64_t stride = 0,
               float *m2 = nullptr);
void release_dist(cr_ctx *c);
uint32_t group_layers(cr_ctx *c, const cr_render_params *p, uint32_t want, uint32_t *m_out);
struct PassTotals {
    uint64_t ctr[sizeof(cr_counters) / sizeof(uint64_t)] = {};
    float ms = 0.f;
    cr_trace_stats ts{};
    void add(const cr_ctx *c) {
        const uint64_t *h = (const uint64_t *)&c->last;
        for (size_t i = 0; i < sizeof(cr_counters) / sizeof(uint64_t); i++) ctr[i] += h[i];
        ms += c->last_ms;
        for (int kind = 0; kind < 4; kind++) {
            ts.launches[kind] += c->last_trace.launches[kind];
            ts.ms[kind] += c->last_trace.ms[kind];
            ts.inner[kind] += c->last_trace.inner[kind];
            ts.leaf[kind] += c->last_trace.leaf[kind];
            ts.tritest[kind] += c->last_trace.tritest[kind];
        }
    }
    void store(cr_ctx *c) const {
        std::memcpy(&c->last, ctr, sizeof(cr_counters));
        c->last_ms = ms;
        c->last_trace = ts;
    }
};
}
```

### chiaroscuro-raytracer_amd/csrc/group.cpp

```cpp
#include "ctx.hpp"

#include <algorithm>
#include <chrono>
#include <cstring>
#include <thread>

namespace crx {

static int nccl_fail(cr_ctx *c, ncclResult_t r, const char *what) {
    return fail(c, CR_E_COMM, std::string(what) + ": " + ncclGetErrorString(r));
}

void release_dist(cr_ctx *c) {
    if (c->comm) ncclCommDestroy(c->comm);
    c->comm = nullptr;
    c->comm_rank = 0;
    c->comm_nranks = 1;
    if (c->d_tiles) hipFree(c->d_tiles);
    if (c->d_gathered) hipFree(c->d_gathered);
    if (c->d_flag) hipFree(c->d_flag);
    c->d_tiles = c->d_gathered = nullptr;
    c->d_flag = nullptr;
    c->tiles_bytes = c->gathered_bytes = c->flag_bytes = 0;
}

static ncclResult_t nccl_settle(ncclComm_t comm) {
    ncclResult_t st = ncclInProgress;
    while (ncclCommGetAsyncError(comm, &st) == ncclSuccess && st == ncclInProgress)
        std::this_thread::sleep_for(std::chrono::microseconds(20));
    return st;
}

static int wait_comm(cr_ctx *c, ncclComm_t comm, hipStream_t st, const char *what) {
    for (;;) {
        const hipError_t q = hipStreamQuery(st);
        if (q == hipSuccess) break;
        if (q != hipErrorNotReady) return hip_fail(c, q, what);
        ncclResult_t ae = ncclSuccess;
        if (comm && ncclCommGetAsyncError(comm, &ae) == ncclSuccess && ae != ncclSuccess && ae != ncclInProgress) {
            ncclCommAbort(comm);
            if (c->comm == comm) c->comm = nullptr;
            return nccl_fail(c, ae, what);
        }
        std::this_thread::sleep_for(std::chrono::microseconds(20));
    }
    ncclResult_t ae = ncclSuccess;
    if (comm && ncclCommGetAsyncError(comm, &ae) == ncclSuccess && ae != ncclSuccess) return nccl_fail(c, ae, what);
    return CR_OK;
}

static int agree(cr_ctx *c, bool ok, hipStream_t st, const char *what) {
    HIPCHK(hipMemsetD32Async((hipDeviceptr_t)c->d_flag, ok ? 1 : 0, 1, st));
    ncclResult_t r = ncclAllReduce(c->d_flag, c->d_flag, 1, ncclInt32, ncclMin, c->comm, st);
    if (r == ncclInProgress) r = nccl_settle(c->comm);
    if (r != ncclSuccess) return nccl_fail(c, r, what);
    if (int rc = wait_comm(c, c->comm, st, what)) return rc;
    int all = 0;
    HIPCHK(hipMemcpy(&all, c->d_flag, sizeof(int), hipMemcpyDeviceToHost));
    if (all == 1) return CR_OK;
    return fail(c, CR_E_INVALID, std::string(what) + ": " +
                                     (ok ? "another rank cannot render this pass group (plan the group with "
                                           "cr_layers_per_group on every rank and agree on the minimum)"
                                         : c->err));
}

static size_t slot_elems(const cr_render_params *p) {
    const size_t T = tile_of(p);
    return (size_t)cr_tiles_for_rank(p, 0) * T * T * 3;
}

static cr::BlendArgs blend_args(const cr_render_params *p, const float *gathered, float *frame) {
    cr::BlendArgs B{};
    B.gathered = gathered;
    B.frame = frame;
    B.xres = p->xres;
    B.yres = p->yres;
    B.tile = tile_of(p);
    B.tiles_x = (p->xres + B.tile - 1) / B.tile;
    B.nranks = p->nranks;
    B.max_tiles = cr_tiles_for_rank(p, 0);
    B.layer = p->layer;
    B.nl = 1;
    return B;
}

static int frame_layers(cr_ctx *c, const cr_camera *cam, const cr_render_params *q, uint32_t nlayers, float *d_frame,
                        hipStream_t st) {
    cr_render_params f = *q;
    f.rank = 0;
    f.nranks = 1;
    uint32_t m = 1;
    if (nlayers > 1 && group_layers(c, &f, nlayers, &m) != nlayers)
        return fail(c, CR_E_INVALID, "layers per pass: the frame does not fit in pieces");
    PassTotals sum;
    for (uint32_t k = 0; k < m; k++) {
        cr_render_params t = f;
        t.rank = k;
        t.nranks = m;
        if (int rc = run_render(c, cam, &t, d_frame, cr::MODE_BLEND, st, nlayers)) return rc;
        sum.add(c);
    }
    sum.store(c);
    return CR_OK;
}

}

using namespace crx;

extern "C" {

int cr_comm_unique_id(uint8_t *out, size_t n) {
    if (!out || n < CR_COMM_ID_BYTES || sizeof(ncclUniqueId) > CR_COMM_ID_BYTES) return CR_E_INVALID;
    ncclUniqueId id;
    if (ncclGetUniqueId(&id) != ncclSuccess) return CR_E_COMM;
    std::memset(out, 0, CR_COMM_ID_BYTES);
    std::memcpy(out, &id, sizeof(id));
    return CR_OK;
}

int cr_comm_init(cr_ctx *c, int nranks, int rank, const uint8_t *id) {
    if (!c) return CR_E_INVALID;
    if (c->device < 0) return fail(c, CR_E_HIP, c->err.empty() ? "no device" : c->err);
    if (nranks < 1 || rank < 0 || rank >= nranks || !id) return fail(c, CR_E_INVALID, "bad nranks/rank/id");
    HIPCHK(hipSetDevice(c->device));
    release_dist(c);
    if (int rr = grow(c, (void **)&c->d_flag, c->flag_bytes, sizeof(int))) return rr;
    ncclUniqueId uid;
    std::memcpy(&uid, id, sizeof(uid));
    ncclComm_t comm = nullptr;
    ncclConfig_t cfg = NCCL_CONFIG_INITIALIZER;
    cfg.blocking = 0;
    ncclResult_t r = ncclCommInitRankConfig(&comm, nranks, uid, rank, &cfg);
    if (r != ncclSuccess && r != ncclInProgress) {
        if (comm) ncclCommAbort(comm);
        return nccl_fail(c, r, "ncclCommInitRankConfig");
    }
    const auto deadline = std::chrono::steady_clock::now() + std::chrono::milliseconds(c->comm_timeout_ms);
    for (;;) {
        ncclResult_t st = ncclInProgress;
        if ((r = ncclCommGetAsyncError(comm, &st)) != ncclSuccess || (st != ncclSuccess && st != ncclInProgress)) {
            ncclCommAbort(comm);
            return nccl_fail(c, r != ncclSuccess ? r : st, "ncclCommInitRankConfig");
        }
        if (st == ncclSuccess) break;
        if (std::chrono::steady_clock::now() > deadline) {
            ncclCommAbort(comm);
            return fail(c, CR_E_COMM, "cr_comm_init: the " + std::to_string(nranks) +
                                          "-rank communicator did not form within " +
                                          std::to_string(c->comm_timeout_ms) + " ms (peers missing)");
        }
        std::this_thread::sleep_for(std::chrono::microseconds(200));
    }
    c->comm = comm;
    c->comm_rank = rank;
    c->comm_nranks = nranks;
    return CR_OK;
}

int cr_comm_destroy(cr_ctx *c) {
    if (!c) return CR_E_INVALID;
    if (c->device >= 0) {
        HIPCHK(hipSetDevice(c->device));
        release_dist(c);
    }
    return CR_OK;
}

int cr_render_dist_device(cr_ctx *c, const cr_camera *cam, const cr_render_params *p, float *d_frame, void *stream) {
    if (!c) return CR_E_INVALID;
    if (c->device < 0) return fail(c, CR_E_HIP, c->err.empty() ? "no device" : c->err);
    if (!p || !cam) return fail(c, CR_E_INVALID, "null camera/params");
    if (!c->comm) return fail(c, CR_E_INVALID, "no communicator (cr_comm_init)");
    cr_render_params q = *p;
    q.rank = (uint32_t)c->comm_rank;
    q.nranks = (uint32_t)c->comm_nranks;
    const bool root = c->comm_rank == 0;
    if (root && !d_frame) return fail(c, CR_E_INVALID, "root needs a frame");
    if (int rc = check_params(c, &q)) return rc;
    HIPCHK(hipSetDevice(c->device));
    hipStream_t st = (hipStream_t)stream;
    if (q.nranks == 1) return run_render(c, cam, &q, d_frame, cr::MODE_BLEND, st);
// ... 384 lines not shown
```

### chiaroscuro-raytracer_amd/csrc/kernels.hpp

```cpp
#pragma once
#include <hip/hip_runtime.h>
#include <stdint.h>

#include "leafcull.hpp"
#include "wfbuilds.hpp"
#include "wfopts.hpp"

namespace cr {

enum { MODE_BLEND = 0, MODE_TILES = 1 };
enum { REC_STRIDE = 3 };
enum { CTR_N = 22, CTR_SLOTS = 112 };
enum { TK_CAMERA = 0, TK_CLOSEST = 1, TK_SHADOW = 2, TK_TAIL = 3, TK_N = 4 };
enum { CTR_TRACE = 24 };
enum { CTR_NEE = 22 };
enum { CTR_DIAG = 40, DIAG_N = 16 };
enum {
    DIAG_ROUNDS = 0,
    DIAG_LANES = 1,
    DIAG_DISTINCT = 2,
    DIAG_RECORDS = 3,
    DIAG_MAXCOUNT = 4,
    DIAG_LANETESTS = 5,
    DIAG_FIT64 = 6,
    DIAG_FIT128 = 7,
    DIAG_UROUNDS = 8,
    DIAG_TESTS = 9,
    DIAG_GEOMISS = 10,
    DIAG_REP1 = 11,
    DIAG_REP4 = 12,
    DIAG_REP8 = 13,
};
enum { CTR_PERF = 64, PERF_N = 12 };
enum {
    PERF_QUERIES = 0,
    PERF_STEPS = 1,
    PERF_LEAVES = 2,
    PERF_MASKS = 3,
    PERF_TESTS = 4,
    PERF_VBYTES = 5,
    PERF_SBYTES = 6,
    PERF_WAVES = 7,
    PERF_DROUNDS = 8,
    PERF_DITERS = 9,
    PERF_DLANES = 10,
    PERF_DTESTS = 11,
};

__host__ __device__ inline uint64_t tex_pad(int w, int nc) { return (uint64_t)(w + 1) * nc + 4; }

__host__ __device__ inline uint32_t tile_slot_column(uint32_t slot, uint32_t tiles_x, uint32_t nranks) {
    const uint32_t row = slot / tiles_x, c = slot - row * tiles_x;
    return nranks > 1 ? (c + row % tiles_x) % tiles_x : c;
}
__host__ __device__ inline uint32_t tile_slot(uint32_t gx, uint32_t gy, uint32_t tiles_x, uint32_t nranks) {
    const uint32_t c = nranks > 1 ? (gx + tiles_x - gy % tiles_x) % tiles_x : gx;
    return gy * tiles_x + c;
}

struct DevScene {
    const uint2 *nodes;
    const uint4 *fat;
    const float4 *recs;
    const float4 *lcullp;
    const uint4 *lcullc;
    LcGrid lcg;
    float db;
    const float4 *tri;
    const float4 *mat_n;
    const float4 *mat_kd;
    const float4 *mat_ke;
    const float2 *mat_uv;
    const uint2 *lights;
    const uint4 *texs;
    const uint8_t *texels;
    uint32_t nlights;
    uint32_t n_nodes;
    float3 bmin, bmax;
};
enum : uint32_t { NODE_BFS = 512 };

struct RenderArgs {
    DevScene S;
    float cam[12];
    uint32_t xres, yres, spp;
    int K;
    float bg[3];
    uint32_t seed, layer;
    uint32_t nl;
    uint64_t layer_stride;
    uint32_t piece_k, piece_m;
    uint32_t rank, nranks, tile, tiles_x;
    uint32_t n_items;
    uint32_t stack_depth;
    int mode;
    float *out;
    unsigned long long *counters;
    uint2 *gstack;
    uint32_t gstride;
    int full_counters;
    int perf_counters;
    int variant;
    uint32_t refill;
    uint32_t refill_shadow;
    uint32_t refill_camera;
    uint32_t s0, s_count, n_work;
    float *samples;
    float *run;
    const float4 *cull;
    const float4 *cull_node;
    int eye_on_split;
    uint32_t diag_kinds;
    int lc_debug;
    uint32_t lc_min;
    uint32_t desc_quorum;
};
inline size_t gstack_bytes(uint32_t depth, uint32_t threads) { return (size_t)depth * threads * 8; }
int launch_sum_samples(const RenderArgs &A, bool first, bool last, hipStream_t st, uint32_t lds = 0, bool staged = true,
                       float *m2 = nullptr, float *run2 = nullptr);

struct NoiseArgs {
    const float *frame, *m2;
    float *err;
    void *stats;
    uint32_t npix, layers;
    float n, threshold, floor;
};
int launch_noise_eval(const NoiseArgs &N, hipStream_t st);

enum : uint32_t { WF_G = 66, WF_XCDS = 8, WF_XSTRIDE = 16, WF_XBASE = 5 * WF_G,
                  WF_CNT = WF_XBASE + 2 * WF_G * WF_XCDS * WF_XSTRIDE };
enum { WF_STATE = 6 };
struct WfArgs {
    uint32_t P;
    uint32_t w0;
    float4 *ray[2];
    uint4 *hit[2];
    float4 *sray;
    uint32_t *sexcl;
    uint32_t *occ;
    uint32_t *cnt;
    float4 *ps;
    float4 *dw;
    uint2 *gstack;
    uint2 *gstack2;
    uint32_t gstride;
    uint32_t *key[2][2], *perm[2][2];
    const uint32_t *order;
    void *sort_tmp;
    size_t sort_tmp_bytes;
    int sort;
    int key_bits;
    int key_bits_pixel;
    uint32_t sort_min;
    uint32_t sort_tile;
    uint32_t dir_res;
    int world_keys;
    uint32_t world_bits;
    uint32_t tail_min;
    float2 *cxy;
    uint32_t xcd;
    int leaf_keys;
    uint32_t resolve_paths;
    uint32_t measure_skip;
    uint32_t leaf_shift;
    uint32_t tail_shadow_gen;
    uint32_t ended_only;
    int tail_overlap;
    uint32_t sort_g1;
    int cam_lean;
    uint32_t dir_res_s;
    int key_bits_s;
    int tail_waves;
    int shade_waves;
// ... 112 lines not shown
```

### chiaroscuro-raytracer_amd/csrc/render_common.hpp

```cpp
#pragma once
#include "device_math.hpp"
#include "kernels.hpp"

namespace cr {

struct Ctr {
    uint32_t closest = 0, shadow = 0, inner = 0, leaf = 0, tritest = 0, hit = 0, texhit = 0, paths = 0, pixels = 0;
    uint32_t wave_desc = 0, wave_tri = 0, wave_round = 0, wave_query = 0;
    uint32_t wave_desc_uniform = 0, wave_tri_uniform = 0;
    uint32_t wave_desc_lines = 0, wave_tri_lines = 0;
    uint32_t leaf_rounds = 0, leaf_distinct = 0, leaf_records = 0, leaf_fit21 = 0, leaf_fit56 = 0;
};
__device__ __forceinline__ uint32_t wave_count(bool pred) { return (uint32_t)__popcll(__ballot(pred)); }
__device__ __forceinline__ uint32_t lane_id() {
    uint32_t l;
    asm volatile("v_mbcnt_lo_u32_b32 %0, -1, 0\n\tv_mbcnt_hi_u32_b32 %0, -1, %0" : "=v"(l));
    return l;
}
__device__ __forceinline__ bool wave_leader() {
    return lane_id() == (uint32_t)(__ffsll((long long)__ballot(1)) - 1);
}

__device__ __forceinline__ void flush_counters(unsigned long long *ctrs, const Ctr &c, uint32_t uniform = 0u) {
    const uint32_t ln = lane_id();
// ... 26 lines not shown
    const float txmin = (S.bmin.x - o.x) * dix, txmax = (S.bmax.x - o.x) * dix;
    const float tymin = (S.bmin.y - o.y) * diy, tymax = (S.bmax.y - o.y) * diy;
    const float tzmin = (S.bmin.z - o.z) * diz, tzmax = (S.bmax.z - o.z) * diz;
    first = std_max(std_max(std_min(txmin, txmax), std_min(tymin, tymax)), std_min(tzmin, tzmax));
    second = std_min(std_min(std_max(txmin, txmax), std_max(tymin, tymax)), std_max(tzmin, tzmax));
}

struct TriRec {
    float4 a;
    float4 b;
    float4 c;
};
__device__ __forceinline__ TriRec load_rec(const DevScene &S, uint32_t ref) {
    const float4 *p = (const float4 *)((const char *)S.recs + (ref * (uint32_t)(16 * REC_STRIDE)));
    return TriRec{p[0], p[1], p[2]};
}
__device__ __forceinline__ uint32_t rec_id(const TriRec &r) { return __float_as_uint(r.a.w); }
__device__ __forceinline__ bool tri_test(f3 o, f3 d, const TriRec &r, float tmax, float &ux, float &uy, float &t) {
    const f3 v0 = ld3(r.a), e1 = ld3(r.b), e2 = ld3(r.c);
    const f3 p = cross(d, e2);
    const float aa = dot(e1, p);
    if (aa < 1.19209290e-7F && aa > -1.19209290e-7F) return false;
    const float f = rcp_rn(aa);
    const f3 sv = sub(o, v0);
    ux = f * dot(sv, p);
    if (ux < 0.f || ux > 1.f) return false;
    const f3 q = cross(sv, e1);
    uy = f * dot(d, q);
    if (uy < 0.f || uy + ux > 1.f) return false;
    t = f * dot(e2, q);
    return t >= 0.f && t < tmax;
}

__device__ __forceinline__ bool tri_test_wave(f3 o, f3 d, const TriRec &r, float tmax, float &ux, float &uy,
                                              float &t, bool live = true) {
    const f3 v0 = ld3(r.a), e1 = ld3(r.b), e2 = ld3(r.c);
    const f3 p = cross(d, e2);
    const float aa = dot(e1, p);
    bool ok = live & !((aa < 1.19209290e-7F) & (aa > -1.19209290e-7F));
    if (!__ballot(ok)) return false;
    const float f = rcp_rn_wave(aa);
    const f3 sv = sub(o, v0);
    ux = f * dot(sv, p);
    ok = ok & !((ux < 0.f) | (ux > 1.f));
    if (!__ballot(ok)) return false;
    const f3 q = cross(sv, e1);
    uy = f * dot(d, q);
    ok = ok & !((uy < 0.f) | (uy + ux > 1.f));
    if (!__ballot(ok)) return false;
    t = f * dot(e2, q);
    return ok & (t >= 0.f) & (t < tmax);
}

__device__ __forceinline__ float split_distance(float split, float oa, float da) { return (split - oa) / da; }

__device__ __forceinline__ f3 tex_lookup(const DevScene &S, int ti, float u, float v) {
    const uint4 t = S.texs[ti];
    const int w = (int)t.x, h = (int)t.y, nc = (int)t.z;
    for (int i = 0; u > 1.f && i < (1 << 24); i++) u -= 1.f;
    for (int i = 0; u < 0.f && i < (1 << 24); i++) u += 1.f;
    for (int i = 0; v > 1.f && i < (1 << 24); i++) v -= 1.f;
    for (int i = 0; v < 0.f && i < (1 << 24); i++) v += 1.f;
    int x = (int)(u * (float)w);
    int y = (int)(v * (float)h);
    long idx = ((long)y * w + x) * nc;
    const long lim = (long)w * h * nc + (long)tex_pad(w, nc);
    if (idx < 0 || idx + 3 > lim) idx = lim - 3 - nc;
    const uint8_t *px = S.texels + t.w + idx;
    return mk((float)px[0] * 0.00392156862f, (float)px[1] * 0.00392156862f, (float)px[2] * 0.00392156862f);
}

__device__ __forceinline__ f3 camera_dir(const RenderArgs &A, uint32_t x, uint32_t y, Rng &rng,
                                         float2 *sxy = nullptr) {
    const f3 lu = mk(A.cam[3], A.cam[4], A.cam[5]), dx = mk(A.cam[6], A.cam[7], A.cam[8]),
             dy = mk(A.cam[9], A.cam[10], A.cam[11]);
    const float uy = rng_uniform(rng, 0.f, 1.f);
    const float ux = rng_uniform(rng, 0.f, 1.f);
    const float sx = (float)x + ux, sy = (float)y + uy;
    if (sxy) *sxy = make_float2(sx, sy);
    return add(add(lu, muls(dx, sx)), muls(dy, sy));
}

__device__ __forceinline__ bool item_pixel(const RenderArgs &A, uint32_t item, uint32_t &x, uint32_t &y) {
    const uint32_t T = A.tile, TT = A.tile * A.tile;
    const uint32_t lt = item / TT, o = item - lt * TT;
    const uint32_t s = A.rank + lt * A.nranks;
    const uint32_t gy = s / A.tiles_x, gx = tile_slot_column(s, A.tiles_x, A.nranks);
    x = gx * T + (o % T);
    y = gy * T + (o / T);
    return x < A.xres && y < A.yres;
}

__device__ __forceinline__ Rng path_rng(const RenderArgs &A, uint32_t pixel, uint32_t s) {
    const uint32_t j = A.nl > 1 ? s / A.spp : 0u;
    return rng_make(A.seed, A.layer + j, pixel, s - j * A.spp);
}

__device__ __forceinline__ void write_pixel(const RenderArgs &A, uint32_t x, uint32_t y, uint32_t item, f3 temp,
                                            uint32_t lj = 0) {
    const float inv = 1.f / (float)A.spp;
    const uint32_t layer = A.layer + lj;
    if (A.mode == MODE_TILES) {
        const f3 m = muls(temp, inv);
        size_t slot = item;
        if (A.piece_m > 1) {
            const uint32_t TT = A.tile * A.tile, lt = item / TT;
            slot = (size_t)(A.piece_k + lt * A.piece_m) * TT + (item - lt * TT);
        }
        float *o = A.out + (size_t)lj * A.layer_stride + 3 * slot;
        o[0] = m.x;
        o[1] = m.y;
        o[2] = m.z;
    } else {
        float *o = A.out + 3 * ((size_t)y * A.xres + x);
        const f3 old = (layer > 1) ? mk(o[0], o[1], o[2]) : mk(0.f, 0.f, 0.f);
        const f3 nw = divs(add(muls(old, (float)(layer - 1)), muls(temp, inv)), (float)layer);
        o[0] = nw.x;
        o[1] = nw.y;
        o[2] = nw.z;
    }
}

struct HitShade {
    f3 p, normal, fcol, direct;
    bool textured;
};
__device__ __forceinline__ HitShade shade_hit(const DevScene &S, f3 origin, uint32_t t, float bx, float by, int k) {
    HitShade h;
    const float4 nrm4 = S.mat_n[t];
    h.normal = ld3(nrm4);
    const float bz = (1.f - bx - by);
    h.p = add(add(muls(ld3(S.tri[3 * t]), bz), muls(ld3(S.tri[3 * t + 1]), bx)), muls(ld3(S.tri[3 * t + 2]), by));
    const float4 kd4 = S.mat_kd[t];
    f3 Kd = ld3(kd4);
    const int ti = __float_as_int(kd4.w);
    h.textured = ti >= 0;
    if (h.textured) {
        const float2 ua = S.mat_uv[3 * t], ub = S.mat_uv[3 * t + 1], uc = S.mat_uv[3 * t + 2];
        Kd = tex_lookup(S, ti, (ua.x * bz + ub.x * bx) + uc.x * by, (ua.y * bz + ub.y * bx) + uc.y * by);
    }
    h.fcol = muls(Kd, (float)0.31830988618379067154);
    const f3 wo = normalize(sub(origin, h.p));
    if (k > 1) {
        h.direct = mk(0.f, 0.f, 0.f);
    } else {
        const bool emissive = __float_as_uint(nrm4.w) != 0u;
        const f3 rad = emissive ? ld3(S.mat_ke[t]) : mk(0.f, 0.f, 0.f);
        h.direct = muls(rad, std_max(0.f, dot(wo, h.normal)));
    }
    return h;
}

struct Nee {
    f3 origin, dir, contrib;
    float distance;
    uint32_t light;
};
__device__ __forceinline__ Nee sample_light(const DevScene &S, f3 p, f3 normal, f3 fcol, Rng &rng) {
    Nee n;
    const uint32_t li = rng_index(rng, S.nlights);
    const uint2 L = S.lights[li];
    n.light = L.x;
    const float v0 = rng_uniform(rng, 0.f, 1.f);
    const float v1 = rng_uniform(rng, 0.f, 1.f - v0);
    const f3 lp = add(add(muls(ld3(S.tri[3 * n.light]), v0), muls(ld3(S.tri[3 * n.light + 1]), v1)),
                      muls(ld3(S.tri[3 * n.light + 2]), 1.f - v0 - v1));
    n.distance = distance3(p, lp);
    n.dir = normalize(sub(lp, p));
    n.origin = add(p, muls(normal, 0.001f));
    const float geometric =
        std_max(0.f, dot(normal, n.dir) * dot(neg(n.dir), ld3(S.mat_n[n.light])) / (1.f + n.distance * n.distance));
    n.contrib = mul(muls(ld3(S.mat_ke[n.light]), geometric * __uint_as_float(L.y) * (float)S.nlights), fcol);
    return n;
// ... 4 lines not shown
```

### chiaroscuro-raytracer_amd/csrc/wavefront.hip

```cpp
#include "append.hpp"
#include "camcull.hpp"
#include "raysort.hpp"
#include "traverse.hpp"

#include <atomic>
#include <thread>

namespace cr {

enum : uint32_t { NO_SLOT = 0xffffffffu, NO_PATH = 0xffffffffu, DEAD_RAY = 1u };
enum : uint32_t { SEXCL_CONT = 0x80000000u };

template <int N>
__device__ __forceinline__ void block_append_chunk(uint32_t *const (&counter)[N], const bool (&pred)[N], uint32_t *lds,
                                                   uint32_t buf, uint32_t C, uint32_t (&cb)[N], uint32_t (&cu)[N],
                                                   uint32_t (&slot)[N]) {
    uint32_t *L = lds + buf * (APP_W + 3u) * N;
    const uint32_t wave = threadIdx.x >> 6;
    uint64_t m[N];
#pragma unroll
    for (int q = 0; q < N; q++) {
        m[q] = __ballot(pred[q]);
        if ((threadIdx.x & 63u) == 0) L[APP_W * q + wave] = (uint32_t)__popcll(m[q]);
    }
// ... 21 lines not shown
                cb[q] = fresh[q];
                cu[q] = tot[q] - room;
            } else {
                cu[q] += tot[q];
            }
        }
    }
    __syncthreads();
#pragma unroll
    for (int q = 0; q < N; q++) {
        const uint32_t i = L[APP_W * q + wave] +
                           __builtin_amdgcn_mbcnt_hi((uint32_t)(m[q] >> 32), __builtin_amdgcn_mbcnt_lo((uint32_t)m[q], 0u));
        const uint32_t room = L[APP_W * N + 3 * q + 1];
        slot[q] = i < room ? L[APP_W * N + 3 * q] + i : L[APP_W * N + 3 * q + 2] + (i - room);
    }
}

__device__ __forceinline__ uint32_t *cnt_closest(const WfArgs &W, uint32_t g) { return W.cnt + g; }
__device__ __forceinline__ uint32_t *cnt_shadow(const WfArgs &W, uint32_t g) { return W.cnt + WF_G + g; }
__device__ __forceinline__ uint32_t *work_closest(const WfArgs &W, uint32_t g) { return W.cnt + 2 * WF_G + g; }
__device__ __forceinline__ uint32_t *work_shadow(const WfArgs &W, uint32_t g) { return W.cnt + 3 * WF_G + g; }

__device__ __forceinline__ uint32_t dir_bin(f3 d, uint32_t res) {
    const float s = fabsf(d.x) + fabsf(d.y) + fabsf(d.z);
    if (!(s > 0.f)) return 0u;
    float u = d.x / s, v = d.z / s;
    if (d.y < 0.f) {
        const float uu = (1.f - fabsf(v)) * (u >= 0.f ? 1.f : -1.f), vv = (1.f - fabsf(u)) * (v >= 0.f ? 1.f : -1.f);
        u = uu;
        v = vv;
    }
    const float h = 0.5f * (float)res;
    const uint32_t bu = (uint32_t)min((int)res - 1, max(0, (int)((u + 1.f) * h)));
    const uint32_t bv = (uint32_t)min((int)res - 1, max(0, (int)((v + 1.f) * h)));
    uint32_t m = 0;
    for (uint32_t b = 0; (1u << b) < res; b++) m |= ((bu >> b) & 1u) << (2 * b + 1) | ((bv >> b) & 1u) << (2 * b);
    return m;
}
__device__ __forceinline__ uint32_t world_key(const RenderArgs &A, const WfArgs &W, f3 o, f3 dir) {
    const DevScene &S = A.S;
    const uint32_t WORLD_BITS = W.world_bits;
    const float sc = (float)(1u << WORLD_BITS);
    const uint32_t qx = (uint32_t)min((int)sc - 1, max(0, (int)((o.x - S.bmin.x) / (S.bmax.x - S.bmin.x) * sc)));
    const uint32_t qy = (uint32_t)min((int)sc - 1, max(0, (int)((o.y - S.bmin.y) / (S.bmax.y - S.bmin.y) * sc)));
    const uint32_t qz = (uint32_t)min((int)sc - 1, max(0, (int)((o.z - S.bmin.z) / (S.bmax.z - S.bmin.z) * sc)));
    uint32_t m = 0;
    for (uint32_t b = 0; b < WORLD_BITS; b++)
        m |= ((qx >> b) & 1u) << (3 * b + 2) | ((qy >> b) & 1u) << (3 * b + 1) | ((qz >> b) & 1u) << (3 * b);
    return m * (W.dir_res * W.dir_res) + dir_bin(dir, W.dir_res);
}
__device__ __forceinline__ uint32_t sort_key(const RenderArgs &A, const WfArgs &W, uint32_t p, f3 dir) {
    const uint32_t item = (W.w0 + p) / A.s_count;
    const uint32_t T = A.tile, TT = T * T, lt = item / TT, o = item - lt * TT, sh = W.sort_tile;
    const uint32_t S = (T + (1u << sh) - 1) >> sh;
    const uint32_t sub = ((o / T) >> sh) * S + ((o % T) >> sh);
    return (lt * S * S + sub) * (W.dir_res * W.dir_res) + dir_bin(dir, W.dir_res);
}

__device__ __forceinline__ void flush_tallies(const RenderArgs &A, unsigned long long *tl) {
    __syncthreads();
    if (threadIdx.x < T_N && tl[threadIdx.x]) atomicAdd(&A.counters[tally_slot(threadIdx.x)], tl[threadIdx.x]);
}

__device__ __forceinline__ void finish_path(const RenderArgs &A, const WfArgs &W, uint32_t p, uint32_t k, f3 tail) {
    f3 acc = tail;
    for (int j = (int)k - 2; j >= 0; j--) {
        const float4 Dj = W.dw[(size_t)(2 * j) * W.P + p];
        const float4 Wj = W.dw[(size_t)(2 * j + 1) * W.P + p];
        acc = add(ld3(Dj), mul(ld3(Wj), acc));
    }
    float *out = A.samples + 3 * (size_t)(W.w0 + p);
    out[0] = acc.x;
    out[1] = acc.y;
    out[2] = acc.z;
}

__device__ __forceinline__ float4 &PS(const WfArgs &W, int slot, uint32_t p) { return W.ps[(size_t)slot * W.P + p]; }
enum { PS_CTL = 5 };
__device__ __forceinline__ void ctl_store(const WfArgs &W, uint32_t p, uint32_t k, const Rng &rng) {
    PS(W, PS_CTL, p) = make_float4(__uint_as_float(k), __uint_as_float(rng.key), __uint_as_float(rng.ctr), 0.f);
}

__host__ __device__ __forceinline__ bool camera_state_lean(const WfArgs &W) { return W.cam_lean && W.P >= W.tail_min; }
__device__ __forceinline__ uint32_t path_key(const RenderArgs &A, const WfArgs &W, uint32_t p) {
    const uint32_t w = W.w0 + p, item = w / A.s_count, s = A.s0 + (w - item * A.s_count);
    uint32_t px = 0, py = 0;
    item_pixel(A, item, px, py);
    return path_rng(A, py * A.xres + px, s).key;
}
__device__ __forceinline__ Rng camera_rng(const RenderArgs &A, const WfArgs &W, uint32_t p) {
    return Rng{path_key(A, W, p), 2u};
}

__global__ void __launch_bounds__(256) wf_camera(RenderArgs A, WfArgs W) {
    __shared__ unsigned long long tl[T_N];
    if (threadIdx.x < T_N) tl[threadIdx.x] = 0;
    __syncthreads();
    for (uint32_t base = blockIdx.x * blockDim.x; base < W.P; base += gridDim.x * blockDim.x) {
        const uint32_t p = base + threadIdx.x;
        const uint32_t w = W.w0 + p;
        uint32_t item = 0, s = 0, px = 0, py = 0;
        bool valid = p < W.P && w < A.n_work;
        if (valid) {
            item = w / A.s_count;
            s = A.s0 + (w - item * A.s_count);
            valid = item_pixel(A, item, px, py);
        }
        tally(tl, T_PATHS, valid);
        if (valid) {
            Rng rng = path_rng(A, py * A.xres + px, s);
            float2 sxy;
            const f3 d = camera_dir(A, px, py, rng, &sxy);
            if (A.cull) W.cxy[p] = sxy;
            if (!camera_state_lean(W)) ctl_store(W, p, 1u, rng);
            W.mark[p] = 0;
            W.ray[1][2 * (size_t)p] = make_float4(A.cam[0], A.cam[1], A.cam[2], __uint_as_float(p));
            W.ray[1][2 * (size_t)p + 1] = pk(d, 0u);
        } else if (p < W.P) {
            W.mark[p] = 0;
            W.ray[1][2 * (size_t)p] = make_float4(0.f, 0.f, 0.f, __uint_as_float(NO_PATH));
            W.ray[1][2 * (size_t)p + 1] = make_float4(0.f, 0.f, 1.f, 0.f);
        }
    }
    if (blockIdx.x == 0 && threadIdx.x == 0) *cnt_closest(W, 1) = W.P;
    flush_tallies(A, tl);
}

enum : uint32_t { SHADOW_VIS = 0u, SHADOW_OCC = 1u };
enum : uint32_t { ENDED_BIT = 0x80000000u };
template <bool FIX>
__device__ __forceinline__ void shadow_store(const WfArgs &W, uint32_t g, uint32_t idx, bool occluded) {
    if (FIX || W.vis_mark) {
        if (!occluded) W.mark[idx & ~ENDED_BIT] = (uint8_t)((g << 2) | 2u | (idx >> 31));
    } else if (W.vis_dw) {
        ((uint32_t *)(W.dw + (size_t)(2 * (g - 1)) * W.P + idx))[3] = occluded ? SHADOW_OCC : SHADOW_VIS;
    } else {
        W.occ[idx] = occluded ? 1u : 0u;
    }
}
__device__ __forceinline__ bool keeps_plus_zero(float v) {
    const uint32_t b = __float_as_uint(v);
    return b != 0x80000000u && (b & 0x7fffffffu) <= 0x7f800000u;
}
__device__ __forceinline__ bool nee_zero(const WfArgs &W, const RenderArgs &A, f3 contrib, f3 direct) {
    return W.nee_skip && !A.full_counters && !A.perf_counters &&
           (__float_as_uint(contrib.x) | __float_as_uint(contrib.y) | __float_as_uint(contrib.z)) == 0u &&
           keeps_plus_zero(direct.x) && keeps_plus_zero(direct.y) && keeps_plus_zero(direct.z);
}
__device__ __forceinline__ bool nee_visible(const WfArgs &W, uint32_t slot) {
    return slot != NO_SLOT && (W.vis_dw ? slot == SHADOW_VIS : W.occ[slot] == 0u);
}

typedef const __attribute__((address_space(4))) char *kargs_ptr;
__device__ __forceinline__ kargs_ptr kargs_here() {
    kargs_ptr p = (kargs_ptr)__builtin_amdgcn_kernarg_segment_ptr();
    asm volatile("" : "+s"(p));
    return p;
}
__device__ __forceinline__ WfArgs kargs_w(kargs_ptr p) {
    WfArgs w;
    __builtin_memcpy(&w, p + KARG_W, sizeof(WfArgs));
    return w;
}
__device__ __forceinline__ uint32_t kargs_g(kargs_ptr p) {
    return *(const __attribute__((address_space(4))) uint32_t *)(p + KARG_G);
}

template <class C>
__global__ void __launch_bounds__(WF_TRACE_BLOCK, C::MINW) wf_trace(RenderArgs A, WfArgs W, uint32_t g) {
    static constexpr bool SHADOW = C::SHADOW, FULL = C::FULL, CAM = C::CAM, PC = C::PC, FIX = C::FIX;
    static constexpr int CULL = C::CULL;
    static_assert(!CULL || (CAM && !SHADOW), "the cull applies to camera rays");
    extern __shared__ uint2 ring_lds[];
    const DevScene &S = A.S;
// ... 143 lines not shown
    if (PC) {
        pc.q = lane == 0 ? issued : 0u;
        pc_flush(A.counters + CTR_PERF + PERF_N * (SHADOW ? TK_SHADOW : (CAM ? TK_CAMERA : TK_CLOSEST)), pc);
    }
    if (FULL) {
        unsigned long long *base = A.counters + CTR_TRACE + 3 * (SHADOW ? TK_SHADOW : (CAM ? TK_CAMERA : TK_CLOSEST));
        const uint32_t v[3] = {c.inner, c.leaf, c.tritest};
#pragma unroll
        for (int i = 0; i < 3; i++) {
            unsigned long long x = v[i];
#pragma unroll
            for (int off = 32; off >= 1; off >>= 1) x += __shfl_xor(x, off, 64);
            if (lane == 0 && x) atomicAdd(&base[i], x);
        }
        diag_flush(A.counters, dg);
    }
}


struct ShadowRay {
    f3 o, d;
    float dist;
    uint32_t light;
};
__device__ __forceinline__ bool shade_path(const RenderArgs &A, const WfArgs &W, uint32_t p, f3 ro, uint4 h,
                                           bool &textured, ShadowRay &sh) {
    const DevScene &S = A.S;
    const float4 ctl = PS(W, PS_CTL, p);
    const uint32_t k = __float_as_uint(ctl.x);
    const HitShade hs = shade_hit(S, ro, h.x, __uint_as_float(h.y), __uint_as_float(h.z), (int)k);
    textured = hs.textured;
    Rng rng{__float_as_uint(ctl.y), __float_as_uint(ctl.z)};
    f3 contrib = mk(0.f, 0.f, 0.f), next = add(hs.p, muls(hs.normal, 0.001f));
    bool nee = false;
    if (S.nlights) {
        const Nee e = sample_light(S, hs.p, hs.normal, hs.fcol, rng);
        contrib = e.contrib;
        next = e.origin;
        sh.o = e.origin;
        sh.d = e.dir;
        sh.dist = e.distance;
        sh.light = e.light;
        nee = !nee_zero(W, A, contrib, hs.direct);
    }
    PS(W, 0, p) = pk(hs.direct, 0u);
    PS(W, 1, p) = pk(hs.fcol, 0u);
    PS(W, 2, p) = pk(hs.normal, 0u);
    ctl_store(W, p, k, rng);
    PS(W, 4, p) = pk(next, 0u);
    PS(W, 3, p) = pk(contrib, NO_SLOT);
    return nee;
}

__device__ __forceinline__ bool bounce_path(const RenderArgs &A, const WfArgs &W, uint32_t p, bool visible, f3 &org,
                                            f3 &wi) {
    const float4 s0 = PS(W, 0, p), s1 = PS(W, 1, p), s2 = PS(W, 2, p), s3 = PS(W, 3, p), ctl = PS(W, PS_CTL, p);
    const uint32_t k = __float_as_uint(ctl.x);
    f3 direct = ld3(s0);
    const f3 fcol = ld3(s1), normal = ld3(s2);
    Rng rng{__float_as_uint(ctl.y), __float_as_uint(ctl.z)};
    if (visible) direct = add(direct, ld3(s3));
    if ((int)k == A.K) {
        finish_path(A, W, p, k, direct);
        return false;
    }
    const float sx = rng_uniform(rng, -1.f, 1.f);
    const float sy = rng_uniform(rng, -1.f, 1.f);
    float pdf;
    sample_wi(normal, sx, sy, wi, pdf);
    const float Kmax = std_max(std_max(fcol.x, fcol.y), fcol.z);
    if (pdf == 0.f || rng_uniform(rng, 0.f, 1.f) > Kmax) {
        finish_path(A, W, p, k, direct);
        return false;
    }
    const float cosine = fabsf(dot(normal, wi));
    const f3 w = divs(muls(fcol, cosine), pdf * Kmax);
    W.dw[(size_t)(2 * (k - 1)) * W.P + p] = pk(direct, 0u);
    W.dw[(size_t)(2 * (k - 1) + 1) * W.P + p] = pk(w, 0u);
    ctl_store(W, p, k + 1, rng);
    org = ld3(PS(W, 4, p));
    return true;
}

__device__ __forceinline__ bool shade_next(const RenderArgs &A, const WfArgs &W, uint32_t p, uint32_t k, f3 ro, uint4 h,
                                           bool &textured, ShadowRay &sh, bool &cont, f3 &org, f3 &wi, uint32_t &ctr,
                                           f3 &direct, bool &skipped) {
    const DevScene &S = A.S;
    const HitShade hs = shade_hit(S, ro, h.x, __uint_as_float(h.y), __uint_as_float(h.z), (int)k);
    textured = hs.textured;
    const bool cam = k == 1u && camera_state_lean(W);
    Rng rng;
    if (cam) {
        rng = camera_rng(A, W, p);
    } else if (W.ctl_ray && k >= 2u) {
        rng = Rng{path_key(A, W, p), ctr};
    } else {
        const float4 ctl = PS(W, PS_CTL, p);
        rng = Rng{__float_as_uint(ctl.y), __float_as_uint(ctl.z)};
    }
    f3 contrib = mk(0.f, 0.f, 0.f), next = add(hs.p, muls(hs.normal, 0.001f));
    bool nee = false;
    if (S.nlights) {
        const Nee e = sample_light(S, hs.p, hs.normal, hs.fcol, rng);
        contrib = e.contrib;
        next = e.origin;
        sh.o = e.origin;
        sh.d = e.dir;
        sh.dist = e.distance;
        sh.light = e.light;
        nee = true;
        skipped = nee_zero(W, A, contrib, hs.direct);
        nee = !skipped;
    }
    cont = false;
    if ((int)k != A.K) {
        const float sx = rng_uniform(rng, -1.f, 1.f);
        const float sy = rng_uniform(rng, -1.f, 1.f);
        float pdf;
        sample_wi(hs.normal, sx, sy, wi, pdf);
        const float Kmax = std_max(std_max(hs.fcol.x, hs.fcol.y), hs.fcol.z);
        if (!(pdf == 0.f || rng_uniform(rng, 0.f, 1.f) > Kmax)) {
            const float cosine = fabsf(dot(hs.normal, wi));
            const f3 w = divs(muls(hs.fcol, cosine), pdf * Kmax);
            W.dw[(size_t)(2 * (k - 1) + 1) * W.P + p] = pk(w, 0u);
            if (W.ctl_ray) ctr = rng.ctr;
            else ctl_store(W, p, k + 1, rng);
            org = next;
            cont = true;
        }
    }
    direct = hs.direct;
    PS(W, 3, p) = pk(W.vis_mark ? add(hs.direct, contrib) : contrib, 0u);
    W.mark[p] = (uint8_t)(W.vis_mark ? (k << 2) | (cont ? 0u : 1u) : (k << 1) | (cont ? 0u : 1u));
    return nee;
}

template <int MINW, bool CH = false, int BS = 256>
__global__ void __launch_bounds__(BS, MINW) wf_shade(RenderArgs A, WfArgs W, uint32_t g) {
    __shared__ unsigned long long tl[T_N];
    __shared__ uint32_t app2[2 * (APP_W + 3) * 2];
    if (threadIdx.x < T_N) tl[threadIdx.x] = 0;
    __syncthreads();
    const uint32_t n = *cnt_closest(W, g);
    const uint32_t C = CH ? W.app_chunk : 0u;
    uint32_t cb[2] = {0u, 0u}, cu[2] = {C, C};
    const float4 *rays = W.ray[g & 1];
    const uint4 *hits = W.hit[g & 1];
    float4 *next_rays = W.ray[(g + 1) & 1];
    uint32_t *const queues[2] = {cnt_shadow(W, g), cnt_closest(W, g + 1)};
    uint32_t it = 0;
    const bool fused = g == 1 && W.cam_fused;
    const uint32_t span = CH ? ((n + gridDim.x - 1) / gridDim.x + blockDim.x - 1) / blockDim.x * blockDim.x : 0u;
    const uint32_t b0 = CH ? blockIdx.x * span : blockIdx.x * blockDim.x;
    const uint32_t b1 = CH ? min(n, b0 + span) : n, bstep = CH ? blockDim.x : gridDim.x * blockDim.x;
    for (uint32_t base = b0; base < b1; base += bstep, it++) {
        const uint32_t i = base + threadIdx.x;
        const bool in = i < n;
        uint4 h = make_uint4(0u, 0u, 0u, 0u);
        float4 r0 = make_float4(0.f, 0.f, 0.f, 0.f);
        uint32_t ctr = 0;
        if (in) {
            h = hits[i];
            if (fused) r0 = make_float4(A.cam[0], A.cam[1], A.cam[2], __uint_as_float(h.x == DEAD_RAY && !h.w ? NO_PATH : i));
            else r0 = rays[2 * (size_t)i];
            if (W.ctl_ray && g >= 2 && h.w) ctr = __float_as_uint(rays[2 * (size_t)i + 1].w);
        }
        const uint32_t p = __float_as_uint(r0.w);
        const bool hit = in && h.w != 0u;
        if (fused) {
            if (in && !hit) W.mark[i] = 0;
            tally(tl, T_PATHS, in && p != NO_PATH);
        }
        bool textured = false, nee = false, cont = false, skipped = false;
        ShadowRay sh = {mk(0.f, 0.f, 0.f), mk(0.f, 0.f, 0.f), 0.f, 0u};
        f3 org = mk(0.f, 0.f, 0.f), wi = mk(0.f, 0.f, 0.f), direct = mk(0.f, 0.f, 0.f);
        if (in && !hit) {
            if (p != NO_PATH) finish_path(A, W, p, g, mk(A.bg[0], A.bg[1], A.bg[2]));
        } else if (hit) {
            nee = shade_next(A, W, p, g, ld3(r0), h, textured, sh, cont, org, wi, ctr, direct, skipped);
        }
        tally(tl, T_SHADOW, skipped);
        tally(tl, T_NEE, skipped);
        const bool want[2] = {nee, cont};
        uint32_t slots[2];
        if (CH) block_append_chunk<2>(queues, want, app2, it & 1u, C, cb, cu, slots);
        else block_append_n<2>(queues, want, app2, it & 1u, slots);
        const uint32_t j = slots[0], jc = slots[1];
        if (hit) W.dw[(size_t)(2 * (g - 1)) * W.P + p] = pk(direct, nee ? j : NO_SLOT);
        if (nee) {
            W.sray[2 * (size_t)j] = pk(sh.o, p);
            W.sray[2 * (size_t)j + 1] = make_float4(sh.d.x, sh.d.y, sh.d.z, sh.dist);
            W.sexcl[j] = sh.light | (cont ? SEXCL_CONT : 0u);
            if (W.sort) {
                W.key[0][0][j] = W.leaf_keys ? ((h.w - 1u) >> W.leaf_shift) * (W.dir_res_s * W.dir_res_s) + dir_bin(sh.d, W.dir_res_s)
                                 : (W.world_keys && g >= (uint32_t)W.world_keys) ? world_key(A, W, sh.o, sh.d)
                                                                                 : sort_key(A, W, p, sh.d);
            }
        }
        if (cont) {
            next_rays[2 * (size_t)jc] = pk(org, p);
            next_rays[2 * (size_t)jc + 1] = pk(wi, W.ctl_ray ? ctr : 0u);
            if (W.sort) {
                W.key[1][0][jc] = W.leaf_keys ? ((h.w - 1u) >> W.leaf_shift) * (W.dir_res * W.dir_res) + dir_bin(wi, W.dir_res)
                                  : (W.world_keys && g >= (uint32_t)W.world_keys) ? world_key(A, W, org, wi)
                                                                                  : sort_key(A, W, p, wi);
            }
        }
        tally(tl, T_HIT, hit);
        tally(tl, T_TEXHIT, textured);
    }
    if (CH) {
        __syncthreads();
        if (threadIdx.x == 0) {
            app2[0] = cb[0] + cu[0];
            app2[1] = cu[0] < C ? C - cu[0] : 0u;
            app2[2] = cb[1] + cu[1];
            app2[3] = cu[1] < C ? C - cu[1] : 0u;
        }
        __syncthreads();
        for (uint32_t q = 0; q < 2; q++) {
            const uint32_t from = app2[2 * q], len = app2[2 * q + 1];
            float4 *rq = q ? next_rays : W.sray;
            for (uint32_t k = threadIdx.x; k < len; k += blockDim.x) {
                const uint32_t j = from + k;
                rq[2 * (size_t)j] = make_float4(0.f, 0.f, 0.f, __uint_as_float(NO_PATH));
                rq[2 * (size_t)j + 1] = make_float4(0.f, 0.f, 1.f, 0.f);
                if (!q) W.sexcl[j] = 0u;
                if (W.sort) {
                    W.key[q][0][j] = 0xffffffffu;
                }
            }
        }
    }
    flush_tallies(A, tl);
}

__device__ __forceinline__ void resolve_path(const RenderArgs &A, const WfArgs &W, uint32_t p, uint32_t g, uint32_t m) {
    const bool ended = m & 1u;
    float4 &dk = W.dw[(size_t)(2 * (g - 1)) * W.P + p];
    if (W.vis_mark) {
        if (m & 2u) {
            const float4 s3 = PS(W, 3, p);
            if (ended) finish_path(A, W, p, g, ld3(s3));
            else dk = s3;
        } else if (ended) {
            finish_path(A, W, p, g, ld3(dk));
        }
        return;
    }
    const float4 d4 = dk;
    const uint32_t slot = __float_as_uint(d4.w);
    f3 direct = ld3(d4);
    if (nee_visible(W, slot)) direct = add(direct, ld3(PS(W, 3, p)));
    if (ended) finish_path(A, W, p, g, direct);
    else dk = pk(direct, 0u);
}

__global__ void __launch_bounds__(256) wf_resolve(RenderArgs A, WfArgs W, uint32_t g) {
    const uint32_t n = *cnt_closest(W, g);
    if (W.resolve_paths && (uint64_t)n * W.resolve_paths >= (uint64_t)W.P) {
        const uint32_t sh = W.vis_mark ? 2u : 1u;
        for (uint32_t p = blockIdx.x * blockDim.x + threadIdx.x; p < W.P; p += gridDim.x * blockDim.x) {
// ... 851 lines not shown
```

### include/chiaro_hip.h

```cpp
#ifndef CHIARO_HIP_H
#define CHIARO_HIP_H

#include <stddef.h>
#include <stdint.h>

#ifdef __cplusplus
extern "C" {
#endif

#define CR_OK 0
#define CR_E_INVALID (-1)
#define CR_E_HIP (-2)
#define CR_E_NOSCENE (-3)
#define CR_E_DEPTH (-4)
#define CR_E_OOM (-5)
#define CR_E_COMM (-6)

typedef struct cr_ctx cr_ctx;

typedef struct {
    float split;
    uint32_t axis;
    uint32_t child_or_first;
    uint32_t count;
// ... 23 lines not shown
    const uint32_t *light_id;
    const float *light_surface;
    uint32_t n_textures;
    const cr_texture *textures;
} cr_scene_desc;

typedef struct {
    float eye[3];
    float left_upper[3];
    float dx[3];
    float dy[3];
} cr_camera;

typedef struct {
    uint32_t xres, yres;
    uint32_t spp;
    int32_t k;
    float background[3];
    uint32_t seed;
    uint32_t layer;
    uint32_t rank, nranks;
    uint32_t tile;
} cr_render_params;

typedef struct {
    uint64_t closest;
    uint64_t shadow;
    uint64_t inner;
    uint64_t leaf;
    uint64_t tritest;
    uint64_t hit;
    uint64_t texhit;
    uint64_t paths;
    uint64_t pixels;
    uint64_t wave_desc;
    uint64_t wave_tri;
    uint64_t wave_round;
    uint64_t wave_query;
    uint64_t wave_desc_uniform;
    uint64_t wave_tri_uniform;
    uint64_t wave_desc_lines;
    uint64_t wave_tri_lines;
    uint64_t leaf_rounds;
    uint64_t leaf_distinct;
    uint64_t leaf_records;
    uint64_t leaf_fit21;
    uint64_t leaf_fit56;
    uint64_t nee_answered;
} cr_counters;

cr_ctx *cr_create(int device);
void cr_destroy(cr_ctx *ctx);
const char *cr_last_error(cr_ctx *ctx);

int cr_upload_scene(cr_ctx *ctx, const cr_scene_desc *desc);

int cr_render(cr_ctx *ctx, const cr_camera *cam, const cr_render_params *p, float *accum_rgb_out);

int cr_set_accumulator(cr_ctx *ctx, uint32_t xres, uint32_t yres, const float *rgb);

int cr_render_device(cr_ctx *ctx, const cr_camera *cam, const cr_render_params *p, float *d_frame, void *stream);

typedef struct cr_tonemap_params {
    float m, s, kl, f, defog, gamma;
} cr_tonemap_params;
void cr_tonemap_setup(float exposure, float defog, float kneeLow, float kneeHigh, float gamma, cr_tonemap_params *out);
int cr_tonemap_device(cr_ctx *ctx, const cr_tonemap_params *t, uint32_t xres, uint32_t yres, const float *d_rgb,
                      uint8_t *d_bytes, void *stream);
int cr_tonemap(cr_ctx *ctx, const cr_tonemap_params *t, uint32_t xres, uint32_t yres, uint8_t *bytes_out);

int cr_render_tiles_device(cr_ctx *ctx, const cr_camera *cam, const cr_render_params *p, float *d_tiles,
                           void *stream);
int cr_blend_tiles_device(cr_ctx *ctx, const cr_render_params *p, const float *d_gathered, float *d_frame,
                          void *stream);
int cr_blend_tiles_layers_device(cr_ctx *ctx, const cr_render_params *p, uint32_t nlayers, const float *d_gathered,
                                 float *d_frame, void *stream);
uint32_t cr_tiles_for_rank(const cr_render_params *p, uint32_t rank);

uint32_t cr_layers_per_pass(cr_ctx *ctx, const cr_render_params *p, uint32_t want);
int cr_render_layers_device(cr_ctx *ctx, const cr_camera *cam, const cr_render_params *p, uint32_t nlayers,
                            float *d_frame, void *stream);
int cr_render_tiles_layers_device(cr_ctx *ctx, const cr_camera *cam, const cr_render_params *p, uint32_t nlayers,
                                  float *d_tiles, void *stream);
int cr_render_layers(cr_ctx *ctx, const cr_camera *cam, const cr_render_params *p, uint32_t nlayers,
                     float *accum_rgb_out);
uint32_t cr_layers_per_group(cr_ctx *ctx, const cr_render_params *p, uint32_t want);
uint32_t cr_scene_triangles(cr_ctx *ctx);
int cr_tile_origin(const cr_render_params *p, uint32_t rank, uint32_t local, uint32_t *x0, uint32_t *y0);

typedef struct cr_noise_params {
    float threshold;
    float floor;
} cr_noise_params;
typedef struct cr_noise_stats {
    uint64_t pixels;
    uint64_t above;
    float max_err;
    uint32_t layers;
} cr_noise_stats;
void cr_noise_struct_sizes(uint32_t *params_bytes, uint32_t *stats_bytes);
int cr_render_layers_noise_device(cr_ctx *ctx, const cr_camera *cam, const cr_render_params *p, uint32_t nlayers,
                                  float *d_frame, float *d_m2, void *stream);
int cr_noise_device(cr_ctx *ctx, uint32_t xres, uint32_t yres, uint32_t layers, uint32_t spp,
                    const cr_noise_params *np, const float *d_frame, const float *d_m2, float *d_err,
                    cr_noise_stats *d_stats, void *stream);
int cr_render_layers_noise(cr_ctx *ctx, const cr_camera *cam, const cr_render_params *p, uint32_t nlayers,
                           float *accum_rgb_out, float *m2_out);
int cr_noise(cr_ctx *ctx, uint32_t xres, uint32_t yres, uint32_t layers, uint32_t spp, const cr_noise_params *np,
             float *err_out, cr_noise_stats *stats_out);
int cr_set_noise_accumulator(cr_ctx *ctx, uint32_t xres, uint32_t yres, const float *m2);
int cr_render_until(cr_ctx *ctx, const cr_camera *cam, const cr_render_params *p, uint32_t min_layers,
                    uint32_t max_layers, uint32_t check_every, const cr_noise_params *np, uint64_t max_above,
                    float *accum_rgb_out, cr_noise_stats *stats_out);

int cr_intersect(cr_ctx *ctx, uint32_t n, const float *orig, const float *dir, uint32_t *hit, uint32_t *tri,
                 float *bary, float *dist);
int cr_intersect_shadow(cr_ctx *ctx, uint32_t n, const float *orig, const float *dir, const float *dist,
                        const uint32_t *light_tri, uint32_t *occluded);
int cr_intersect_device(cr_ctx *ctx, uint32_t n, const float *d_orig, const float *d_dir, uint32_t *d_hit,
                        uint32_t *d_tri, float *d_bary, float *d_dist, void *stream);
int cr_intersect_shadow_device(cr_ctx *ctx, uint32_t n, const float *d_orig, const float *d_dir,
                               const float *d_dist, const uint32_t *d_light_tri, uint32_t *d_occluded,
                               void *stream);

int cr_get_counters(cr_ctx *ctx, cr_counters *out);
float cr_last_kernel_ms(cr_ctx *ctx);
typedef struct cr_trace_stats {
    uint64_t launches[4];
    double ms[4];
    uint64_t inner[4], leaf[4], tritest[4];
    uint64_t chunked_shades;
} cr_trace_stats;
int cr_get_trace_stats(cr_ctx *ctx, cr_trace_stats *out);
int cr_set_option(cr_ctx *ctx, const char *key, int64_t value);
int cr_get_diag(cr_ctx *ctx, uint64_t *out, int n);
int cr_get_perf(cr_ctx *ctx, uint64_t *out, int n);
int cr_trace_build_available(int build);
int cr_last_trace_build(cr_ctx *ctx);
int cr_synchronize(cr_ctx *ctx);


#define CR_COMM_ID_BYTES 128
int cr_comm_unique_id(uint8_t *id_out, size_t id_bytes);
int cr_comm_init(cr_ctx *ctx, int nranks, int rank, const uint8_t *id);
int cr_comm_destroy(cr_ctx *ctx);
int cr_render_dist_device(cr_ctx *ctx, const cr_camera *cam, const cr_render_params *p, float *d_frame,
                          void *stream);
int cr_render_dist_layers_device(cr_ctx *ctx, const cr_camera *cam, const cr_render_params *p, uint32_t nlayers,
                                 float *d_frame, void *stream);

typedef struct cr_group cr_group;
int cr_device_count(void);
cr_group *cr_group_create(int ngpus, const int *devices);
void cr_group_destroy(cr_group *g);
const char *cr_group_last_error(cr_group *g);
int cr_group_size(cr_group *g);
int cr_group_ok(cr_group *g);
int cr_group_upload_scene(cr_group *g, const cr_scene_desc *desc);
int cr_group_set_option(cr_group *g, const char *key, int64_t value);
int cr_group_render(cr_group *g, const cr_camera *cam, const cr_render_params *p, float *accum_rgb_out);
int cr_group_render_layers(cr_group *g, const cr_camera *cam, const cr_render_params *p, uint32_t nlayers,
                           float *accum_rgb_out);
int cr_group_get_counters(cr_group *g, cr_counters *out);
int cr_group_rank_ms(cr_group *g, float *ms_out);
cr_ctx *cr_group_ctx(cr_group *g, int rank);
int cr_group_set_accumulator(cr_group *g, uint32_t xres, uint32_t yres, const float *rgb);
// ... 7 lines not shown
```

Before: 2489 Mray/s.

## Precompute per-row tile coordinates and add contiguous block-ordered render pieces

Adds a host-built, cached device table of per-tile-row pixel origins so kernels map a work item to its pixel with one table load instead of div/mod slot arithmetic. It also adds an option to split a frame into contiguous pieces, optionally walked in 8x8 tile blocks, instead of interleaved rank-style pieces, which is meant to improve spatial coherence and cache locality of rays within a pass. Interleaving stays the default, so the block ordering only runs when that option is turned off. The cost is an extra global load per item, a host table rebuild plus H2D copy whenever the key changes, and more code paths.

```diff
diff --git a/chiaroscuro-raytracer_amd/chiaroscuro_amd/__init__.py b/chiaroscuro-raytracer_amd/chiaroscuro_amd/__init__.py
--- a/chiaroscuro-raytracer_amd/chiaroscuro_amd/__init__.py
+++ b/chiaroscuro-raytracer_amd/chiaroscuro_amd/__init__.py
@@ -174,7 +174,8 @@
                "cr_render_tiles_layers_device", "cr_render_layers", "cr_scene_triangles", "cr_layers_per_group",
                "cr_blend_tiles_layers_device", "cr_render_dist_layers_device", "cr_group_render_layers",
                "cr_noise_struct_sizes", "cr_render_layers_noise_device", "cr_noise_device", "cr_render_layers_noise",
-               "cr_noise", "cr_set_noise_accumulator", "cr_render_until")
+               "cr_noise", "cr_set_noise_accumulator", "cr_render_until", "cr_layers_per_pass_piece",
+               "cr_render_layers_piece_device", "cr_piece_tile_origin")
 HOST_SYMBOLS = ("chiaro_last_error", "chiaro_scene_create", "chiaro_scene_info_get", "chiaro_scene_destroy",
                 "chiaro_model_create", "chiaro_model_load", "chiaro_model_num_meshes", "chiaro_model_num_triangles",
                 "chiaro_model_num_textures", "chiaro_model_triangles", "chiaro_model_texture",
@@ -232,6 +233,11 @@
     _sig(hip, "cr_render_layers_device", C.c_int, [P, C.POINTER(CrCamera), C.POINTER(CrRenderParams), C.c_uint32, P, P])
     _sig(hip, "cr_render_tiles_layers_device", C.c_int,
          [P, C.POINTER(CrCamera), C.POINTER(CrRenderParams), C.c_uint32, P, P])
+    _sig(hip, "cr_layers_per_pass_piece", C.c_uint32, [P, C.POINTER(CrRenderParams), C.c_uint32, C.c_uint32])
+    _sig(hip, "cr_render_layers_piece_device", C.c_int,
+         [P, C.POINTER(CrCamera), C.POINTER(CrRenderParams), C.c_uint32, C.c_uint32, C.c_uint32, P, P])
+    _sig(hip, "cr_piece_tile_origin", C.c_int, [C.POINTER(CrRenderParams), C.c_uint32, C.c_uint32, C.c_uint32, C.c_uint32,
+                                                C.c_uint32, C.POINTER(C.c_uint32), C.POINTER(C.c_uint32)])
     _sig(hip, "cr_blend_tiles_device", C.c_int, [P, C.POINTER(CrRenderParams), P, P, P])
     _sig(hip, "cr_blend_tiles_layers_device", C.c_int, [P, C.POINTER(CrRenderParams), C.c_uint32, P, P, P])
     _sig(hip, "cr_tiles_for_rank", C.c_uint32, [C.POINTER(CrRenderParams), C.c_uint32])
@@ -591,6 +597,23 @@
                                                     C.c_void_p(d_frame_ptr), C.c_void_p(stream)),
                   "cr_render_layers_device")
 
+    def layers_per_pass_piece(self, p, want: int, npieces: int) -> int:
+        return int(libs()[0].cr_layers_per_pass_piece(self._c, C.byref(p), want, npieces))
+
+    def render_layers_piece_device(self, cam, p, nlayers: int, piece: int, npieces: int, d_frame_ptr: int,
+                                   stream: int = 0):
+        self._chk(libs()[0].cr_render_layers_piece_device(self._c, C.byref(cam), C.byref(p), nlayers, piece, npieces,
+                                                          C.c_void_p(d_frame_ptr), C.c_void_p(stream)),
+                  "cr_render_layers_piece_device")
+
+    @staticmethod
+    def piece_tile_origin(p: CrRenderParams, rank: int, order: int, piece: int, npieces: int, local: int):
+        x0, y0 = C.c_uint32(0), C.c_uint32(0)
+        if libs()[0].cr_piece_tile_origin(C.byref(p), int(rank), int(order), int(piece), int(npieces), int(local),
+                                          C.byref(x0), C.byref(y0)):
+            raise ValueError("cr_piece_tile_origin: no such tile")
+        return x0.value, y0.value
+
     def render_tiles_layers_device(self, cam, p, nlayers: int, d_tiles_ptr: int, stream: int = 0):
         self._chk(libs()[0].cr_render_tiles_layers_device(self._c, C.byref(cam), C.byref(p), nlayers,
                                                           C.c_void_p(d_tiles_ptr), C.c_void_p(stream)),
diff --git a/chiaroscuro-raytracer_amd/chiaroscuro_amd/tiles.py b/chiaroscuro-raytracer_amd/chiaroscuro_amd/tiles.py
--- a/chiaroscuro-raytracer_amd/chiaroscuro_amd/tiles.py
+++ b/chiaroscuro-raytracer_amd/chiaroscuro_amd/tiles.py
@@ -115,8 +115,12 @@
         for nl in range(want, 0, -1):
             for m in range(1, max_pieces + 1):
                 q = _with_layer(params, params.layer)
-                q.rank, q.nranks = 0, m
-                if self.dev.layers_per_pass(q, nl) == nl:
+                if hasattr(self.dev, "layers_per_pass_piece"):
+                    fit = self.dev.layers_per_pass_piece(q, nl, m)
+                else:
+                    q.rank, q.nranks = 0, m
+                    fit = self.dev.layers_per_pass(q, nl)
+                if fit == nl:
                     return nl, m
         return 1, 1
 
@@ -154,8 +158,11 @@
         if L.nranks == 1:
             for k in range(pieces):
                 q = _with_layer(params, params.layer)
-                q.rank, q.nranks = k, pieces
-                self.dev.render_layers_device(cam, q, nlayers, self.frame.data_ptr(), stream)
+                if hasattr(self.dev, "render_layers_piece_device"):
+                    self.dev.render_layers_piece_device(cam, q, nlayers, k, pieces, self.frame.data_ptr(), stream)
+                else:
+                    q.rank, q.nranks = k, pieces
+                    self.dev.render_layers_device(cam, q, nlayers, self.frame.data_ptr(), stream)
                 self._stats_add()
             return
         if pieces != 1:
diff --git a/chiaroscuro-raytracer_amd/csrc/cabi.cpp b/chiaroscuro-raytracer_amd/csrc/cabi.cpp
--- a/chiaroscuro-raytracer_amd/csrc/cabi.cpp
+++ b/chiaroscuro-raytracer_amd/csrc/cabi.cpp
@@ -3,6 +3,7 @@
 #include "wfplan.hpp"
 
 #include <algorithm>
+#include <array>
 #include <cmath>
 #include <cstdio>
 #include <cstring>
@@ -107,6 +108,7 @@
     A.nranks = p->nranks;
     A.tile = tile_of(p);
     A.tiles_x = (p->xres + A.tile - 1) / A.tile;
+    A.tile_xy = nullptr;
     A.n_items = cr_tiles_for_rank(p, p->rank) * A.tile * A.tile;
     A.stack_depth = c->stack_depth;
     A.mode = mode;
@@ -139,7 +141,8 @@
 }
 
 int run_render(cr_ctx *c, const cr_camera *cam, const cr_render_params *p, float *out, int mode, hipStream_t st,
-               uint32_t nl, uint32_t piece_k, uint32_t piece_m, uint64_t stride, float *m2) {
+               uint32_t nl, uint32_t piece_k, uint32_t piece_m, uint64_t stride, float *m2, uint32_t cut_k,
+               uint32_t cut_m) {
     if (!cam || !out) return fail(c, CR_E_INVALID, "null camera/output");
     if (m2 && mode != cr::MODE_BLEND) return fail(c, CR_E_INVALID, "moments are tracked for blended frames only");
     int rc = check_params(c, p);
@@ -156,6 +159,43 @@
         A.piece_k = piece_k;
         A.piece_m = piece_m;
         A.layer_stride = stride;
+    }
+    uint32_t first = 0, order = cr::TILE_ORDER_ROWS;
+    if (cut_m > 1) {
+        const uint32_t share = cr_tiles_for_rank(p, p->rank);
+        if (piece_m > 1 || !cr::piece_valid(share, cut_k, cut_m))
+            return fail(c, CR_E_INVALID, "bad piece: piece < pieces <= the share's tiles");
+        first = cr::piece_first(share, cut_k, cut_m);
+        order = p->nranks == 1 && mode == cr::MODE_BLEND && !cr::wf_chunked(*c, c->n_tris) ? c->wf_piece_order
+                                                                                         : (uint32_t)cr::TILE_ORDER_ROWS;
+        A.rank = p->rank + first * p->nranks;
+        if (mode == cr::MODE_TILES) A.out += (size_t)first * A.tile * A.tile * 3;
+        A.n_items = (cr::piece_first(share, cut_k + 1, cut_m) - first) * A.tile * A.tile;
+    }
+    {
+        const uint32_t count = A.n_items / (A.tile * A.tile), ty = (p->yres + A.tile - 1) / A.tile;
+        const std::array<uint32_t, 8> key{p->xres, p->yres, A.tile, p->rank, p->nranks, order, first, count};
+        const void *had = c->d_tile_xy;
+        const size_t rows = (size_t)count * A.tile;
+        const int r = grow(c, &c->d_tile_xy, c->tile_xy_bytes, rows * sizeof(uint4));
+        if (c->d_tile_xy != had) c->tile_xy_key = {};
+        if (r) return r;
+        if (key != c->tile_xy_key) {
+            c->tile_xy_key = {};
+            c->h_tile_xy.resize(rows);
+            for (uint32_t t = 0; t < count; t++) {
+                uint32_t gx = 0, gy = 0;
+                cr::piece_tile_xy(order, first, t, p->rank, p->nranks, A.tiles_x, ty, gx, gy);
+                const uint32_t x0 = gx * A.tile, in_x = std::min(A.tile, p->xres - x0);
+                for (uint32_t r = 0; r < A.tile; r++) {
+                    const uint32_t y = gy * A.tile + r;
+                    c->h_tile_xy[(size_t)t * A.tile + r] = make_uint4(x0, y, y * p->xres + x0, y < p->yres ? in_x : 0u);
+                }
+            }
+            HIPCHK(hipMemcpyAsync(c->d_tile_xy, c->h_tile_xy.data(), rows * sizeof(uint4), hipMemcpyHostToDevice, st));
+            c->tile_xy_key = key;
+        }
+        A.tile_xy = (const uint4 *)c->d_tile_xy;
     }
     if (c->kernel == 2 && !c->full_counters && !cr::wf_variant_available(A.variant))
         return fail(c, CR_E_INVALID, "trace build " + std::to_string(A.variant) +
@@ -254,6 +294,22 @@
     return CR_OK;
 }
 
+int run_render_piece(cr_ctx *c, const cr_camera *cam, const cr_render_params *p, float *out, int mode, hipStream_t st,
+                     uint32_t nl, uint32_t k, uint32_t m, float *m2) {
+    if (!p || !cr::piece_valid(cr_tiles_for_rank(p, p->rank), k, m))
+        return fail(c, CR_E_INVALID, "bad piece: piece < pieces <= the share's tiles");
+    if (m == 1) return run_render(c, cam, p, out, mode, st, nl, 0, 1, 0, m2);
+    if (!c->wf_piece_interleave) return run_render(c, cam, p, out, mode, st, nl, 0, 1, 0, m2, k, m);
+    const uint32_t N = p->nranks;
+    cr_render_params t = *p;
+    t.rank = p->rank + k * N;
+    t.nranks = N * m;
+    if (mode != cr::MODE_TILES) return run_render(c, cam, &t, out, mode, st, nl, 0, 1, 0, m2);
+    if (N == 1) return fail(c, CR_E_INVALID, "interleaved pieces of a whole frame's tile buffer");
+    const uint64_t stride = (uint64_t)cr_tiles_for_rank(p, 0) * tile_of(p) * tile_of(p) * 3;
+    return run_render(c, cam, &t, out, mode, st, nl, k, m, stride);
+}
+
 }
 
 using namespace crx;
@@ -316,6 +372,7 @@
         if (c->d_wf) hipFree(c->d_wf);
         if (c->d_cull) hipFree(c->d_cull);
         if (c->d_cull_node) hipFree(c->d_cull_node);
+        if (c->d_tile_xy) hipFree(c->d_tile_xy);
         if (c->d_counters) hipFree(c->d_counters);
         if (c->ev0) hipEventDestroy(c->ev0);
         for (int i = 0; i < 2 * c->tev.cap; i++) hipEventDestroy(c->tev.ev[i]);
@@ -657,10 +714,7 @@
     uint32_t m = 1;
     const uint32_t nl = crx::group_layers(c, &g, std::min(LAYER_GROUP, want), &m);
     for (uint32_t k = 0; k < m; k++) {
-        cr_render_params t = g;
-        t.rank = k;
-        t.nranks = m;
-        if (int rc = crx::run_render(c, cam, &t, c->d_accum, cr::MODE_BLEND, c->stream, nl, 0, 1, 0, m2)) return rc;
+        if (int rc = crx::run_render_piece(c, cam, &g, c->d_accum, cr::MODE_BLEND, c->stream, nl, k, m, m2)) return rc;
         sum.add(c);
     }
     *nl_out = nl;
@@ -900,6 +954,35 @@
     return run_render(c, cam, p, d_frame, cr::MODE_BLEND, (hipStream_t)stream, nlayers);
 }
 
+uint32_t cr_layers_per_pass_piece(cr_ctx *c, const cr_render_params *p, uint32_t want, uint32_t npieces) {
+    if (!p || !cr::piece_valid(cr_tiles_for_rank(p, p->rank), 0, npieces)) return 1;
+    cr_render_params t = *p;
+    t.nranks = p->nranks * npieces;
+    return cr_layers_per_pass(c, &t, want);
+}
+
+int cr_render_layers_piece_device(cr_ctx *c, const cr_camera *cam, const cr_render_params *p, uint32_t nlayers,
+                                  uint32_t piece, uint32_t npieces, float *d_frame, void *stream) {
+    if (!c) return CR_E_INVALID;
+    if (c->device < 0) return fail(c, CR_E_HIP, c->err.empty() ? "no device" : c->err);
+    if (!p || p->nranks != 1) return fail(c, CR_E_INVALID, "cr_render_layers_piece_device: the whole frame (nranks 1)");
+    return run_render_piece(c, cam, p, d_frame, cr::MODE_BLEND, (hipStream_t)stream, nlayers, piece, npieces);
+}
+
+int cr_piece_tile_origin(const cr_render_params *p, uint32_t rank, uint32_t order, uint32_t piece, uint32_t npieces,
+                         uint32_t local, uint32_t *x0, uint32_t *y0) {
+    const uint32_t n = cr_tiles_for_rank(p, rank);
+    if (!p || !x0 || !y0 || order >= cr::TILE_ORDERS || !cr::piece_valid(n, piece, npieces)) return CR_E_INVALID;
+    const uint32_t first = cr::piece_first(n, piece, npieces);
+    if (local >= cr::piece_first(n, piece + 1, npieces) - first) return CR_E_INVALID;
+    const uint32_t T = tile_of(p), tx = (p->xres + T - 1) / T, ty = (p->yres + T - 1) / T;
+    uint32_t gx = 0, gy = 0;
+    cr::piece_tile_xy(order, first, local, rank, p->nranks, tx, ty, gx, gy);
+    *x0 = gx * T;
+    *y0 = gy * T;
+    return CR_OK;
+}
+
 int cr_render_tiles_layers_device(cr_ctx *c, const cr_camera *cam, const cr_render_params *p, uint32_t nlayers,
                                   float *d_tiles, void *stream) {
     if (!c) return CR_E_INVALID;
@@ -909,15 +992,9 @@
     uint32_t m = 1;
     if (group_layers(c, p, nlayers, &m) != nlayers)
         return fail(c, CR_E_INVALID, "layers per pass: the rank's share does not fit in pieces");
-    const uint64_t stride = (uint64_t)cr_tiles_for_rank(p, 0) * tile_of(p) * tile_of(p) * 3;
     PassTotals sum;
     for (uint32_t k = 0; k < m; k++) {
-        cr_render_params t = *p;
-        t.rank = p->rank + k * p->nranks;
-        t.nranks = p->nranks * m;
-        if (cr_tiles_for_rank(&t, t.rank) == 0) continue;
-        if (int rc = run_render(c, cam, &t, d_tiles, cr::MODE_TILES, (hipStream_t)stream, nlayers, k, m, stride))
-            return rc;
+        if (int rc = run_render_piece(c, cam, p, d_tiles, cr::MODE_TILES, (hipStream_t)stream, nlayers, k, m)) return rc;
         sum.add(c);
     }
     sum.store(c);
@@ -1318,6 +1395,8 @@
     else if (!std::strcmp(key, "wf_paths") && v >= 4096 && v <= (1ll << 30)) c->wf_paths = (uint32_t)v;
     else if (!std::strcmp(key, "wf_lanes") && (v == 1 || v == 2)) c->wf_lanes = (int)v;
     else if (!std::strcmp(key, "wf_xcd") && v >= 0 && v <= 7) c->wf_xcd = (uint32_t)v;
+    else if (!std::strcmp(key, "wf_piece_interleave") && (v == 0 || v == 1)) c->wf_piece_interleave = (int)v;
+    else if (!std::strcmp(key, "wf_piece_order") && v >= 0 && v < cr::TILE_ORDERS) c->wf_piece_order = (uint32_t)v;
     else if (!std::strcmp(key, "wf_leaf_keys") && (v == 0 || v == 1)) c->wf_leaf_keys = (int)v;
     else if (!std::strcmp(key, "wf_resolve_paths") && v >= 0 && v <= 64) c->wf_resolve_paths = (uint32_t)v;
     else if (!std::strcmp(key, "wf_measure_skip") && v >= 0 && v <= 3) c->wf_measure_skip = (uint32_t)v;
diff --git a/chiaroscuro-raytracer_amd/csrc/ctx.hpp b/chiaroscuro-raytracer_amd/csrc/ctx.hpp
--- a/chiaroscuro-raytracer_amd/csrc/ctx.hpp
+++ b/chiaroscuro-raytracer_amd/csrc/ctx.hpp
@@ -6,6 +6,7 @@
 #include <hip/hip_runtime.h>
 #include <rccl/rccl.h>
 
+#include <array>
 #include <cstring>
 #include <string>
 #include <vector>
@@ -43,6 +44,10 @@
     size_t accum2_elems = 0;
     void *d_run2 = nullptr, *d_err = nullptr, *d_nstats = nullptr;
     size_t run2_bytes = 0, err_bytes = 0, nstats_bytes = 0;
+    void *d_tile_xy = nullptr;
+    size_t tile_xy_bytes = 0;
+    std::vector<uint4> h_tile_xy;
+    std::array<uint32_t, 8> tile_xy_key{};
     void *d_cull = nullptr;
     size_t cull_bytes = 0;
     void *d_cull_node = nullptr;
@@ -66,6 +71,8 @@
     uint32_t sum_lds = 0;
     int sum_staged = 1;
     uint32_t node_bfs = cr::NODE_BFS;
+    int wf_piece_interleave = 1;
+    uint32_t wf_piece_order = cr::TILE_ORDER_BLOCKS;
     ncclComm_t comm = nullptr;
     int comm_rank = 0, comm_nranks = 1;
     uint32_t comm_timeout_ms = 120000;
@@ -101,7 +108,9 @@
 int grow(cr_ctx *c, void **buf, size_t &cap, size_t need);
 int run_render(cr_ctx *c, const cr_camera *cam, const cr_render_params *p, float *out, int mode, hipStream_t st,
                uint32_t nl = 1, uint32_t piece_k = 0, uint32_t piece_m = 1, uint64_t stride = 0,
-               float *m2 = nullptr);
+               float *m2 = nullptr, uint32_t cut_k = 0, uint32_t cut_m = 1);
+int run_render_piece(cr_ctx *c, const cr_camera *cam, const cr_render_params *p, float *out, int mode, hipStream_t st,
+                     uint32_t nl, uint32_t k, uint32_t m, float *m2 = nullptr);
 void release_dist(cr_ctx *c);
 uint32_t group_layers(cr_ctx *c, const cr_render_params *p, uint32_t want, uint32_t *m_out);
 struct PassTotals {
diff --git a/chiaroscuro-raytracer_amd/csrc/group.cpp b/chiaroscuro-raytracer_amd/csrc/group.cpp
--- a/chiaroscuro-raytracer_amd/csrc/group.cpp
+++ b/chiaroscuro-raytracer_amd/csrc/group.cpp
@@ -94,10 +94,7 @@
         return fail(c, CR_E_INVALID, "layers per pass: the frame does not fit in pieces");
     PassTotals sum;
     for (uint32_t k = 0; k < m; k++) {
-        cr_render_params t = f;
-        t.rank = k;
-        t.nranks = m;
-        if (int rc = run_render(c, cam, &t, d_frame, cr::MODE_BLEND, st, nlayers)) return rc;
+        if (int rc = run_render_piece(c, cam, &f, d_frame, cr::MODE_BLEND, st, nlayers, k, m)) return rc;
         sum.add(c);
     }
     sum.store(c);
diff --git a/chiaroscuro-raytracer_amd/csrc/kernels.hpp b/chiaroscuro-raytracer_amd/csrc/kernels.hpp
--- a/chiaroscuro-raytracer_amd/csrc/kernels.hpp
+++ b/chiaroscuro-raytracer_amd/csrc/kernels.hpp
@@ -58,6 +58,40 @@
     return gy * tiles_x + c;
 }
 
+__host__ __device__ inline uint32_t piece_first(uint32_t n, uint32_t k, uint32_t npieces) {
+    return (uint32_t)((uint64_t)k * n / npieces);
+}
+__host__ __device__ inline bool piece_valid(uint32_t n, uint32_t k, uint32_t npieces) {
+    return npieces >= 1 && k < npieces && (npieces == 1 || npieces <= n);
+}
+enum : uint32_t { TILE_ORDER_ROWS = 0, TILE_ORDER_BLOCKS = 1, TILE_ORDERS = 2, TILE_BLOCK = 8 };
+__host__ __device__ inline uint32_t tile_order_local(uint32_t order, uint32_t j, uint32_t tiles_x, uint32_t tiles_y,
+                                                     uint32_t nranks) {
+    if (order != TILE_ORDER_BLOCKS || nranks > 1) return j;
+    const uint32_t B = TILE_BLOCK, band = tiles_x * B;
+    const uint32_t br = j / band, r = j - br * band;
+    const uint32_t rows = tiles_y - br * B, h = rows < B ? rows : B;
+    const uint32_t bc = r / (B * h), r2 = r - bc * (B * h);
+    const uint32_t cols = tiles_x - bc * B, w = cols < B ? cols : B;
+    const uint32_t ly = r2 / w, lx = r2 - ly * w;
+    return (br * B + ly) * tiles_x + bc * B + lx;
+}
+__host__ __device__ inline uint32_t tile_order_pos(uint32_t order, uint32_t local, uint32_t tiles_x, uint32_t tiles_y,
+                                                   uint32_t nranks) {
+    if (order != TILE_ORDER_BLOCKS || nranks > 1) return local;
+    const uint32_t B = TILE_BLOCK, gy = local / tiles_x, gx = local - gy * tiles_x;
+    const uint32_t br = gy / B, bc = gx / B;
+    const uint32_t rows = tiles_y - br * B, h = rows < B ? rows : B;
+    const uint32_t cols = tiles_x - bc * B, w = cols < B ? cols : B;
+    return br * (tiles_x * B) + bc * (B * h) + (gy - br * B) * w + (gx - bc * B);
+}
+__host__ __device__ inline void piece_tile_xy(uint32_t order, uint32_t first, uint32_t t, uint32_t rank, uint32_t nranks,
+                                              uint32_t tiles_x, uint32_t tiles_y, uint32_t &gx, uint32_t &gy) {
+    const uint32_t s = rank + tile_order_local(order, first + t, tiles_x, tiles_y, nranks) * nranks;
+    gy = s / tiles_x;
+    gx = tile_slot_column(s, tiles_x, nranks);
+}
+
 struct DevScene {
     const uint2 *nodes;
     const uint4 *fat;
@@ -90,6 +124,7 @@
     uint32_t nl;
     uint64_t layer_stride;
     uint32_t piece_k, piece_m;
+    const uint4 *tile_xy;
     uint32_t rank, nranks, tile, tiles_x;
     uint32_t n_items;
     uint32_t stack_depth;
diff --git a/chiaroscuro-raytracer_amd/csrc/render_common.hpp b/chiaroscuro-raytracer_amd/csrc/render_common.hpp
--- a/chiaroscuro-raytracer_amd/csrc/render_common.hpp
+++ b/chiaroscuro-raytracer_amd/csrc/render_common.hpp
@@ -132,13 +132,22 @@
 }
 
 __device__ __forceinline__ bool item_pixel(const RenderArgs &A, uint32_t item, uint32_t &x, uint32_t &y) {
+    const uint32_t T = A.tile, row = item / T, col = item - row * T;
+    const uint4 e = A.tile_xy[row];
+    x = e.x + col;
+    y = e.y;
+    return col < e.w;
+}
+__device__ __forceinline__ uint32_t item_pixel_index(const RenderArgs &A, uint32_t item) {
+    const uint32_t T = A.tile, row = item / T;
+    return A.tile_xy[row].z + (item - row * T);
+}
+__device__ __forceinline__ uint32_t item_pixel_index_rows(const RenderArgs &A, uint32_t item) {
     const uint32_t T = A.tile, TT = A.tile * A.tile;
     const uint32_t lt = item / TT, o = item - lt * TT;
     const uint32_t s = A.rank + lt * A.nranks;
     const uint32_t gy = s / A.tiles_x, gx = tile_slot_column(s, A.tiles_x, A.nranks);
-    x = gx * T + (o % T);
-    y = gy * T + (o / T);
-    return x < A.xres && y < A.yres;
+    return (gy * T + (o / T)) * A.xres + gx * T + (o % T);
 }
 
 __device__ __forceinline__ Rng path_rng(const RenderArgs &A, uint32_t pixel, uint32_t s) {
diff --git a/chiaroscuro-raytracer_amd/csrc/wavefront.hip b/chiaroscuro-raytracer_amd/csrc/wavefront.hip
--- a/chiaroscuro-raytracer_amd/csrc/wavefront.hip
+++ b/chiaroscuro-raytracer_amd/csrc/wavefront.hip
@@ -127,14 +127,14 @@
 }
 
 __host__ __device__ __forceinline__ bool camera_state_lean(const WfArgs &W) { return W.cam_lean && W.P >= W.tail_min; }
+template <bool ROWS = false>
 __device__ __forceinline__ uint32_t path_key(const RenderArgs &A, const WfArgs &W, uint32_t p) {
     const uint32_t w = W.w0 + p, item = w / A.s_count, s = A.s0 + (w - item * A.s_count);
-    uint32_t px = 0, py = 0;
-    item_pixel(A, item, px, py);
-    return path_rng(A, py * A.xres + px, s).key;
-}
+    return path_rng(A, ROWS ? item_pixel_index_rows(A, item) : item_pixel_index(A, item), s).key;
+}
+template <bool ROWS = false>
 __device__ __forceinline__ Rng camera_rng(const RenderArgs &A, const WfArgs &W, uint32_t p) {
-    return Rng{path_key(A, W, p), 2u};
+    return Rng{path_key<ROWS>(A, W, p), 2u};
 }
 
 __global__ void __launch_bounds__(256) wf_camera(RenderArgs A, WfArgs W) {
@@ -444,6 +444,7 @@
     return true;
 }
 
+template <bool ROWS = false>
 __device__ __forceinline__ bool shade_next(const RenderArgs &A, const WfArgs &W, uint32_t p, uint32_t k, f3 ro, uint4 h,
                                            bool &textured, ShadowRay &sh, bool &cont, f3 &org, f3 &wi, uint32_t &ctr,
                                            f3 &direct, bool &skipped) {
@@ -453,9 +454,9 @@
     const bool cam = k == 1u && camera_state_lean(W);
     Rng rng;
     if (cam) {
-        rng = camera_rng(A, W, p);
+        rng = camera_rng<ROWS>(A, W, p);
     } else if (W.ctl_ray && k >= 2u) {
-        rng = Rng{path_key(A, W, p), ctr};
+        rng = Rng{path_key<ROWS>(A, W, p), ctr};
     } else {
         const float4 ctl = PS(W, PS_CTL, p);
         rng = Rng{__float_as_uint(ctl.y), __float_as_uint(ctl.z)};
@@ -539,7 +540,7 @@
         if (in && !hit) {
             if (p != NO_PATH) finish_path(A, W, p, g, mk(A.bg[0], A.bg[1], A.bg[2]));
         } else if (hit) {
-            nee = shade_next(A, W, p, g, ld3(r0), h, textured, sh, cont, org, wi, ctr, direct, skipped);
+            nee = shade_next<CH>(A, W, p, g, ld3(r0), h, textured, sh, cont, org, wi, ctr, direct, skipped);
         }
         tally(tl, T_SHADOW, skipped);
         tally(tl, T_NEE, skipped);
diff --git a/include/chiaro_hip.h b/include/chiaro_hip.h
--- a/include/chiaro_hip.h
+++ b/include/chiaro_hip.h
@@ -129,6 +129,11 @@
                             float *d_frame, void *stream);
 int cr_render_tiles_layers_device(cr_ctx *ctx, const cr_camera *cam, const cr_render_params *p, uint32_t nlayers,
                                   float *d_tiles, void *stream);
+uint32_t cr_layers_per_pass_piece(cr_ctx *ctx, const cr_render_params *p, uint32_t want, uint32_t npieces);
+int cr_render_layers_piece_device(cr_ctx *ctx, const cr_camera *cam, const cr_render_params *p, uint32_t nlayers,
+                                  uint32_t piece, uint32_t npieces, float *d_frame, void *stream);
+int cr_piece_tile_origin(const cr_render_params *p, uint32_t rank, uint32_t order, uint32_t piece, uint32_t npieces,
+                         uint32_t local, uint32_t *x0, uint32_t *y0);
 int cr_render_layers(cr_ctx *ctx, const cr_camera *cam, const cr_render_params *p, uint32_t nlayers,
                      float *accum_rgb_out);
 uint32_t cr_layers_per_group(cr_ctx *ctx, const cr_render_params *p, uint32_t want);
```

Measured after the change: 2497 Mray/s (median of 6 runs). About the same (+0.3%).
